# tansey/functionalmf

Measured on AMD Instinct MI355X. Metric: Gibbs sweeps/sec (full W+V update) at (512,256,64) K=5; % HBM roofline, higher is better.
Workload: dtype f64; 1 GPU; gaussian_btf c3 (512,256,64,4) nembeds=5 tf_order=2 complete data, W+V update, rng=device; burn_in_sweeps=10, step_loop=C side (btf_wv_steps: one call queues the K steps), v_sampler=spectral, likelihood_form=complete, parallelism=rows(W)/cols(V) x1

## Files before the change

### functionalmf_amd/_native.py

```python
import ctypes as C
import os
import subprocess
import sys

import numpy as np

HERE = os.path.dirname(os.path.abspath(__file__))
ROOT = os.path.dirname(HERE)
CSRC = os.path.join(HERE, "csrc")
LIB_PATH = os.environ.get("BTF_LIB_PATH") or os.path.join(HERE, "libbtf_hip.so")
UNITS = [(os.path.join(CSRC, "btf_%s.hip" % name), suffix) for name, suffix in [
    ("abi", "_abi.o"), ("analysis", "_analysis.o"), ("criteria", "_crit.o"), ("nmf", "_nmf.o"), ("gass_ep", "_gass_ep.o"),
    ("gamma_grid", "_gamma_grid.o"), ("diag", "_diag.o"), ("predict", "_predict.o"), ("functionals", "_functionals.o"),
    ("fold_in", "_fold_in.o"), ("loo", "_loo.o"), ("ranking", "_ranking.o"), ("assoc", "_assoc.o"), ("monotone", "_monotone.o"),
    ("gg_criteria", "_gg_criteria.o"), ("gg_predict", "_gg_predict.o")]]
SOURCES = [src for src, _ in UNITS]
HEADERS = sorted(os.path.join(CSRC, f) for f in os.listdir(CSRC) if f.endswith(".h")) + \
    [os.path.join(ROOT, "include", "btf.h")]

BTF_OK, BTF_EINVAL, BTF_EHIP, BTF_ENOTPD, BTF_ESTATE = 0, 1, 2, 3, 4
COMPAT = {"reference": 0, "exact": 1}
KERNEL_NAMES = ["stats", "w_accum", "w_solve", "v_accum", "v_banded", "gram", "products", "sse", "pg_draw", "nb_loglik",
                "prior_band", "gram_eig", "hyper", "ess", "criteria"]
COMM_ID_BYTES = 128
# ... 72 lines not shown
                                          _c_ip, C.c_int] + [_c_dp] * 10 + [C.c_longlong]),
    "btf_posterior_monotone": (C.c_int, [C.c_int] * 6 + [_c_dp, _c_dp, C.c_int, C.c_int, _c_dp, C.c_int, _c_dp, _c_ip, _c_dp, _c_dp]),
    "btf_collect_monotone": (C.c_int, [_ctx, C.c_int, _c_dp, _c_dp, C.c_int, C.c_int, C.c_int, _c_dp, C.c_int, _c_dp, _c_ip, _c_dp, _c_dp]),
    "btf_fold_in_rows": (C.c_int, [C.c_int] * 7 + [_c_dp] * 7 + [C.c_uint64, C.c_int, C.c_int64, _c_dp, _c_dp, C.c_int, _c_dp, C.c_int,
                                   _c_dp, _c_dp]),
    "btf_collect_fold_in": (C.c_int, [_ctx, C.c_int, C.c_int, C.c_int] + [_c_dp] * 4 + [C.c_uint64, C.c_int, C.c_int64, _c_dp, _c_dp,
                                                                                       C.c_int, _c_dp, C.c_int, _c_dp, _c_dp]),
    "btf_diag_eval": (C.c_int, [C.c_int, C.c_int, C.c_int, C.c_int, C.c_int, C.c_int, C.c_int, C.POINTER(_c_dp), C.POINTER(_c_dp),
                                C.POINTER(_ctx), C.c_int, _c_dp]),
    "btf_collect_begin": (C.c_int, [_ctx, C.c_int]),
    "btf_collect": (C.c_int, [_ctx, C.c_int]),
    "btf_collect_schedule": (C.c_int, [_ctx, C.c_int, C.c_int, C.c_int]),
    "btf_collect_end": (C.c_int, [_ctx, C.c_int, _c_dp, _c_dp, _c_dp, _c_dp]),
    "btf_collect_summary": (C.c_int, [_ctx, C.c_int, C.c_int, _c_dp, C.c_int, _c_dp, _c_dp]),
    "btf_crit_set_data": (C.c_int, [_ctx, C.c_int, _c_dp, _c_dp, _c_dp, _c_dp]),
    "btf_crit_set_logsum": (C.c_int, [_ctx, C.c_int, _c_dp]),
    "btf_crit_eval": (C.c_int, [_ctx, C.c_int, C.c_int, C.c_double, C.c_int, _c_dp, _c_dp, _c_dp, C.c_int, _c_dp, _c_dp, _c_dp]),
    "btf_crit_loo": (C.c_int, [_ctx, C.c_int, C.c_int, C.c_double, C.c_int, _c_dp, _c_dp, _c_dp, C.c_int, _c_dp, C.c_int, _c_dp, _c_dp,
                               _c_dp]),
    "btf_predict_batch": (C.c_int, [C.c_int, C.c_int, C.c_int64, _c_dp, _c_dp, C.c_uint64, _c_dp]),
    "btf_predict_eval": (C.c_int, [_ctx, C.c_int, C.c_double, C.c_int, _c_dp, _c_dp, _c_dp, C.c_int, _c_dp, _c_dp, C.c_int, C.c_int,
                                   C.c_uint64, _c_dp, C.c_int, _c_ip, C.c_int] + [_c_dp] * 11),
    "btf_predict_gg_eval": (C.c_int, [_ctx, C.c_int, _c_dp, _c_dp, _c_dp, C.c_int, C.c_int, C.c_uint64, _c_dp, C.c_int, _c_ip, C.c_int] +
                            [_c_dp] * 11),
    "btf_predict_gg_batch": (C.c_int, [C.c_int, C.c_int64, _c_dp, C.c_int, _c_dp, _c_dp, _c_dp, C.c_uint64, _c_dp, _c_ip]),
    "btf_nmf_create": (C.c_int, [C.POINTER(C.c_void_p), C.c_int, C.c_int, C.c_int, C.c_int, C.c_int, C.c_int, _c_dp,
                                 C.POINTER(C.c_uint8), C.c_double]),
    "btf_nmf_run": (C.c_int, [C.c_void_p, _c_dp, _c_dp, C.c_int, C.c_int, C.c_int, C.c_int, C.c_double, C.c_int, _c_ip, _c_dp,
                              _c_dp]),
    "btf_nmf_set_bounds": (C.c_int, [C.c_void_p, C.c_double]),
    "btf_nmf_set_row_features": (C.c_int, [C.c_void_p, C.c_int, _c_dp, C.POINTER(C.c_uint8)]),
    "btf_nmf_run_bounded": (C.c_int, [C.c_void_p, _c_dp, _c_dp, _c_dp, C.c_int, C.c_int, C.c_int, C.c_int, C.c_double, C.c_int,
                                      _c_ip, _c_dp, _c_dp, C.POINTER(C.c_uint8), _c_ip]),
    "btf_nmf_destroy": (None, [C.c_void_p]),
    "btf_nmf_pav": (C.c_int, [C.c_int, C.c_int, C.c_int, C.c_int, C.c_int, _c_dp, _c_dp]),
    "btf_sync": (C.c_int, [_ctx]),
    "btf_ess_begin": (C.c_int, [_ctx, C.c_int, _c_dp, C.c_uint64, C.c_double, C.c_int]),
    "btf_ess_eval": (C.c_int, [_ctx, C.c_int, C.c_double, C.c_int, C.c_int, _c_dp]),
    "btf_ess_run": (C.c_int, [_ctx, C.c_int, C.c_int, C.c_int, _c_dp, C.c_uint64, C.c_int, C.c_double, C.c_int]),
    "btf_ess_info": (C.c_int, [_ctx, _c_ip, _c_dp]),
    "btf_mvn_banded": (C.c_int, [C.c_int, C.c_int, C.c_int, C.c_int, _c_dp, _c_dp, _c_dp, C.c_uint64,
                                 C.c_double, C.c_int, _c_dp, _c_ip]),
    "btf_set_profiling": (C.c_int, [_ctx, C.c_int]),
    "btf_kernel_times": (C.c_int, [_ctx, _c_dp, C.POINTER(C.c_int64)]),
    "btf_set_tuning": (C.c_int, [_ctx, C.c_int, C.c_int]),
    "btf_set_option": (C.c_int, [_ctx, C.c_int, C.c_int]),
    "btf_sym_eig": (C.c_int, [C.c_int, C.c_int, C.c_int, _c_dp, _c_dp, _c_dp]),
    "btf_read_probe": (C.c_int, [C.c_int, C.c_size_t, C.c_int, _c_dp]),
    "btf_queue_Tau2": (C.c_int, [_ctx, C.c_uint64, C.c_double]),
    "btf_queue_lam2": (C.c_int, [_ctx, C.c_uint64, C.c_int]),
    "btf_gibbs_sweeps": (C.c_int, [_ctx, C.c_int, C.c_uint64, C.c_uint64, C.c_int, C.c_double, C.c_double, C.c_double,
                                   C.c_double, C.c_double, C.c_double, C.c_int]),
    "btf_wv_steps": (C.c_int, [_ctx, C.c_int, C.c_uint64, C.c_uint64, C.c_int, C.c_double, C.c_int]),
    "btf_gass_set_constraints": (C.c_int, [_ctx, _c_dp, C.c_int, _c_dp, C.c_int]),
    "btf_gass_begin": (C.c_int, [_ctx, C.c_int, C.c_int, _c_dp, _c_dp, C.c_uint64, C.c_double, C.c_int, C.c_int]),
    "btf_gass_grid": (C.c_int, [_ctx, C.c_int, _c_ip, C.POINTER(C.c_uint8), _c_dp, _c_dp]),
    "btf_gass_eval": (C.c_int, [_ctx, C.c_int, _c_dp, _c_ip, _c_dp]),
    "btf_gass_commit": (C.c_int, [_ctx, C.c_int, _c_dp, _c_ip]),
    "btf_gass_select": (C.c_int, [_ctx, C.c_int, C.c_uint64, _c_ip]),
    "btf_gass_run": (C.c_int, [_ctx, C.c_int, C.c_int, C.c_uint64, C.c_int, C.c_double, C.c_int]),
    "btf_gass_set_ep": (C.c_int, [_ctx, _c_dp, _c_dp]),
    "btf_gass_set_row_features": (C.c_int, [_ctx, C.c_int, C.POINTER(C.c_uint8), _c_dp]),
    "btf_gass_set_U": (C.c_int, [_ctx, _c_dp]),
    "btf_gass_get_U": (C.c_int, [_ctx, _c_dp]),
    "btf_mvn_dense": (C.c_int, [C.c_int, C.c_int, C.c_int, _c_dp, C.c_int, _c_dp, _c_dp, _c_dp, C.c_uint64, C.c_double, C.c_int,
                                _c_dp, _c_ip]),
    "btf_get_likelihood_form": (C.c_int, [_ctx, _c_ip]),
    "btf_get_draw_counters": (C.c_int, [_ctx, C.POINTER(C.c_uint64), C.POINTER(C.c_uint64)]),
    "btf_set_draw_counters": (C.c_int, [_ctx, C.c_uint64, C.c_uint64]),
    "btf_get_accum_bytes_per_cell": (C.c_int, [_ctx, _c_dp]),
    "btf_get_V_sampler": (C.c_int, [_ctx, _c_ip]),
    "btf_queue_scalars": (C.c_int, [_ctx, C.c_uint64, C.c_int, C.c_double, C.c_double, C.c_double, C.c_double, _c_ip]),
    "btf_host_selftest": (C.c_int, []),
    "btf_set_likelihood_param": (C.c_int, [_ctx, C.c_int, C.c_double]),
    "btf_set_likelihood_table": (C.c_int, [_ctx, C.c_int, _c_dp, _c_dp, _c_dp, C.c_int]),
    "btf_set_data_logsum": (C.c_int, [_ctx, _c_dp, _c_dp, C.c_int]),
    "btf_comm_fork": (C.c_int, [_ctx, C.c_void_p]),
    "btf_comm_join": (C.c_int, [_ctx, C.c_void_p]),
    "btf_comm_unique_id": (C.c_int, [C.POINTER(C.c_ubyte), C.c_int]),
    "btf_comm_block": (C.c_int, [C.c_int, C.c_int, C.c_int, _c_ip, _c_ip]),
    "btf_comm_init": (C.c_int, [_ctx, C.c_int, C.c_int, C.POINTER(C.c_ubyte), C.c_int]),
    "btf_comm_rehearse": (C.c_int, [_ctx, C.c_int, C.c_int]),
    "btf_peer_export": (C.c_int, [_ctx, C.POINTER(C.c_ubyte), C.c_int]),
    "btf_peer_init": (C.c_int, [_ctx, C.c_int, C.c_int, C.POINTER(C.c_ubyte), C.c_int]),
    "btf_comm_destroy": (C.c_int, [_ctx]),
    "btf_comm_info": (C.c_int, [_ctx, _c_ip]),
    "btf_allgather_W": (C.c_int, [_ctx]),
    "btf_allgather_V": (C.c_int, [_ctx]),
    "btf_allreduce_sse": (C.c_int, [_ctx]),
    "btf_allreduce_sum": (C.c_int, [_ctx, _c_dp, C.c_int]),
    "btf_set_gathered_W": (C.c_int, [_ctx, _c_dp]),
    "btf_set_gathered_V": (C.c_int, [_ctx, _c_dp]),
}


class BTFError(RuntimeError):
    def __init__(self, code, msg, index=-1):
        super().__init__("btf error %d: %s" % (code, msg))
        self.code = code
        self.index = index


class NotPositiveDefiniteError(BTFError, np.linalg.LinAlgError):
    """Raised where the reference raises LinAlgError (W step, factor.py:357) and
    where it would loop forever after the jitter retries (fast_mvn.py:69-72)."""

# ... 114 lines not shown
```

### functionalmf_amd/csrc/btf_abi.hip

```cpp
#include "../../include/btf.h"
#include "btf_kernels.h"
#include "btf_banded_fast.h"
#include "btf_banded_twist.h"
#include "btf_banded_chunk.h"
#include "btf_spectral.h"
#include "btf_gass.h"
#include "btf_gass_ep.h"
#include "btf_gass_features.h"
#include "btf_gamma_grid.h"
#include "btf_fused.h"
#include "btf_functionals.h"
#include "btf_instances.h"
#include "btf_comm.h"
#include "btf_ctx.h"
#include <hip/hip_ext.h>
#include <unistd.h>

#include <algorithm>
#include <atomic>
#include <climits>
#include <cmath>
#include <cstdio>
#include <cstdlib>
#include <cstring>
// ... 134 lines not shown
      if (cnt > VS_MAXE) { c->st_dense_ok = false; break; }
      for (int u = 0; u < cnt; ++u) { drow[e * VS_MAXE + u] = row[ptr[e] + u]; dcoef[e * VS_MAXE + u] = coef[ptr[e] + u]; }
    }
    if ((rc = dev_alloc(c, &c->st_drow, drow.size()))) return rc;
    if ((rc = dev_alloc(c, &c->st_dcoef, dcoef.size()))) return rc;
    HIPCHK(c, hipMemcpy(c->st_drow, drow.data(), drow.size() * sizeof(int), hipMemcpyHostToDevice));
    HIPCHK(c, hipMemcpy(c->st_dcoef, dcoef.data(), dcoef.size() * sizeof(double), hipMemcpyHostToDevice));
  }
  return BTF_OK;
}

inline int unr3_min_rpb() {
  static const int v = [] { const char* e = std::getenv("BTF_UNR3_RPB"); return e ? std::atoi(e) : 2048; }();
  return v;
}
inline bool lean_on() {
  static const bool v = [] { const char* e = std::getenv("BTF_ACC_LEAN"); return !e || std::atoi(e) != 0; }();
  return v;
}
template <int K>
void launch_accum(btf_ctx* c, int kid, int mode, const double* X, const double* Cx, const unsigned char* C8, const double* U,
                  const int* srcmap, int Rdim, int ld, int rpb, int nch, EigSide side = EigSide{nullptr, 0, 0, nullptr},
                  EigSideCols sidec = EigSideCols{nullptr, 0, CurveLists{nullptr, nullptr, nullptr}, nullptr, 0.0, nullptr},
                  TauSide tau = TauSide{}, GramSide gram = GramSide{},
                  ChunkMap cm = ChunkMap{0, 0, INT_MAX, 0, 0, 0}, SweepSide sw = SweepSide{},
                  const FuseW* fw = nullptr, const FuseV* fv = nullptr) {
  if (cm.row_end == 0) cm.row_end = Rdim;
  {
    static const double min_mb = [] { const char* e = std::getenv("BTF_NT_MIN_MB"); return e ? std::atof(e) : 100.0; }();
    cm.nt = (double)Rdim * (double)ld * 8.0 >= min_mb * 1048576.0 ? 1 : 0;
  }
#ifdef BTF_ACC_STAMPS
  cm.stamps = c->acc_stamps;
#endif
  Prof p(c, kid);
  const int cpw = TAU_SIDE_CPW;
  cm.nside = (sw.sc.hyp ? 1 : 0) + (sw.lam.hyp ? 1 : 0) + (side.out ? 1 + eig_side_groups(sidec.ncols, acc_waves(K, mode)) : 0) +
             (tau.Tau2 ? (tau.M + cpw - 1) / cpw : 0) + (gram.gpart ? gram.nblocks : 0) + (gram.sum_src ? 1 : 0) + (fw ? fw->owners : 0);
  dim3 grid((ld / ACC_TILE) * nch + cm.nside);
  if (fw || fv) {
    const bool unr3 = rpb >= unr3_min_rpb();
    if constexpr (K == 8) {
      if (unr3 && fw) { p.launch(accum_kernel<K, 0, 16, double, double, 3, 2, FUSE_W>, grid, dim3(16 * WAVE), 0, X, Cx, U, srcmap, c->part, Rdim, ld, rpb, side, sidec, tau, gram, cm, sw, *fw); return; }
      if (unr3 && fv) { p.launch(accum_kernel<K, 0, 16, double, double, 3, 2, FUSE_V>, grid, dim3(16 * WAVE), 0, X, Cx, U, srcmap, c->part, Rdim, ld, rpb, side, sidec, tau, gram, cm, sw, *fv); return; }
    }
    if constexpr (K <= 8) {
      if (fw) p.launch(accum_kernel<K, 0, 16, double, double, 0, 2, FUSE_W>, grid, dim3(16 * WAVE), 0, X, Cx, U, srcmap, c->part, Rdim, ld, rpb, side, sidec, tau, gram, cm, sw, *fw);
      else {
        const bool df_on = c->fused_dataflow != 0;
        FuseV f2 = *fv;
        constexpr int RG = K < 4 ? 4 : (K > 6 ? 6 : K);
        f2.dataflow = (df_on && f2.a.pband && f2.pimg && !f2.cnt && !f2.hp.flag && K <= 6 &&
                       vf_df_fits(f2.a.T, K, f2.a.TF, f2.a.nD, 16, RG)) ? 1 : 0;

        if constexpr (K <= 6) {
          if (f2.dataflow) { p.launch(accum_kernel<K, 0, 16, double, double, 0, 2, FUSE_VDF>, grid, dim3(16 * WAVE), 0, X, Cx, U, srcmap, c->part, Rdim, ld, rpb, side, sidec, tau, gram, cm, sw, f2); return; }
        }
        p.launch(accum_kernel<K, 0, 16, double, double, 0, 2, FUSE_V>, grid, dim3(16 * WAVE), 0, X, Cx, U, srcmap, c->part, Rdim, ld, rpb, side, sidec, tau, gram, cm, sw, f2);
      }
    }
    return;
  }
  const signed char* A8 = (mode >= 1 && !C8 && X == c->A_wT) ? c->A8_wT : ((mode >= 1 && !C8 && X == c->A_v) ? c->A8_v : nullptr);
  if (A8) {
    if (mode == 2) p.launch(accum_kernel<K, 2, acc_waves(K, 2), double, signed char>, grid, dim3(acc_waves(K, 2) * WAVE), 0, A8, Cx, U, srcmap, c->part, Rdim, ld, rpb, side, sidec, tau, gram, cm, sw, FuseNone{});
    else p.launch(accum_kernel<K, 1, acc_waves(K, 1), double, signed char>, grid, dim3(acc_waves(K, 1) * WAVE), 0, A8, Cx, U, srcmap, c->part, Rdim, ld, rpb, side, sidec, tau, gram, cm, sw, FuseNone{});
    return;
  }
  if (mode >= 1 && C8) {
    if (mode == 2) p.launch(accum_kernel<K, 2, acc_waves(K, 2), unsigned char>, grid, dim3(acc_waves(K, 2) * WAVE), 0, X, C8, U, srcmap, c->part, Rdim, ld, rpb, side, sidec, tau, gram, cm, sw, FuseNone{});
    else p.launch(accum_kernel<K, 1, acc_waves(K, 1), unsigned char>, grid, dim3(acc_waves(K, 1) * WAVE), 0, X, C8, U, srcmap, c->part, Rdim, ld, rpb, side, sidec, tau, gram, cm, sw, FuseNone{});
  } else if (mode == 2) p.launch(accum_kernel<K, 2>, grid, dim3(acc_waves(K, 2) * WAVE), 0, X, Cx, U, srcmap, c->part, Rdim, ld, rpb, side, sidec, tau, gram, cm, sw, FuseNone{});
  else if (mode == 1) p.launch(accum_kernel<K, 1>, grid, dim3(acc_waves(K, 1) * WAVE), 0, X, Cx, U, srcmap, c->part, Rdim, ld, rpb, side, sidec, tau, gram, cm, sw, FuseNone{});
  else if (K <= 8 && acc_waves(K, 0) == 16 && rpb < unr3_min_rpb() && !tau.Tau2 && !sw.sc.hyp && !sw.lam.hyp && lean_on()) {
    if constexpr (K <= 8) p.launch(accum_kernel<K, 0, 16, double, double, 0, 2, FUSE_LEAN>, grid, dim3(16 * WAVE), 0, X, Cx, U, srcmap, c->part, Rdim, ld, rpb, side, sidec, tau, gram, cm, sw, FuseNone{});
  }
  else if (K >= 10 && ACC_WAVES != acc_waves(10, 0) && !side.out && rpb < unr3_min_rpb()) {
    if constexpr (K >= 10) p.launch(accum_kernel<K, 0, ACC_WAVES>, grid, dim3(ACC_WAVES * WAVE), 0, X, Cx, U, srcmap, c->part, Rdim, ld, rpb, side, sidec, tau, gram, cm, sw, FuseNone{});
  }
  else if (rpb >= unr3_min_rpb()) p.launch(accum_kernel<K, 0, acc_waves(K, 0), double, double, 3>, grid, dim3(acc_waves(K, 0) * WAVE), 0, X, Cx, U, srcmap, c->part, Rdim, ld, rpb, side, sidec, tau, gram, cm, sw, FuseNone{});
  else p.launch(accum_kernel<K, 0>, grid, dim3(acc_waves(K, 0) * WAVE), 0, X, Cx, U, srcmap, c->part, Rdim, ld, rpb, side, sidec, tau, gram, cm, sw, FuseNone{});
}
struct PgPasses { bool flat, series, frac; int mode; };
PgPasses pg_passes(const btf_ctx* c) {
  PgPasses p{false, false, false, c->pg_mode};
  if (c->counts && p.mode == PG_MODE_DEFAULT) p.mode = PG_MODE_SERIES_ALL;
  if (p.mode == PG_MODE_SERIES_ALL) { p.series = true; return p; }
  if (p.mode == PG_MODE_EXACT_ALL) { p.flat = c->pg_has_small || c->pg_has_big; p.frac = c->pg_has_frac; }
  else { p.flat = c->pg_has_small; p.series = c->pg_has_big || c->pg_has_frac; }
  if (!p.flat && !p.series && !p.frac) p.series = true;
  return p;
}
template <int K>
void launch_pg(btf_ctx* c, const double* B, double* out, const double* Lf, const double* Uf, int nl, int ld, int Rdim,
               unsigned long long base, unsigned long long stride_r, unsigned long long stride_l, unsigned long long seed) {
  const int gx = (nl + PG_THREADS - 1) / PG_THREADS;
  int nrb = std::max(1, std::min(Rdim, 4096 / std::max(1, gx)));
  const int rpb = (Rdim + nrb - 1) / nrb;
  nrb = (Rdim + rpb - 1) / rpb;
  const PgPasses ps = pg_passes(c);
  int fill = 1;
  if (ps.flat) {
    Prof p(c, BTF_K_PG);
    const int rpx = round_up(rpb, PGX_CPL);
    p.launch(pgx_kernel<K, PGX_CPL>, dim3(gx, (Rdim + rpx - 1) / rpx), dim3(256), pgx_rows_lds(PGX_CPL), B, out, Lf, Uf, nl, ld, Rdim,
             rpx, base, stride_r, stride_l, seed, ps.mode, fill);
    fill = 0;
  }
  if (ps.series) {
    Prof p(c, BTF_K_PG);
    p.launch(pg_kernel<K, PG_PATH_SERIES>, dim3(gx, nrb), dim3(PG_THREADS), 0, B, out, Lf, Uf, nl, ld, Rdim, rpb, base, stride_r, stride_l, seed, ps.mode, fill);
    fill = 0;
  }
  if (ps.frac) {
    Prof p(c, BTF_K_PG);
    p.launch(pg_kernel<K, PG_PATH_EXACT>, dim3(gx, nrb), dim3(PG_THREADS), 0, B, out, Lf, Uf, nl, ld, Rdim, rpb, base, stride_r, stride_l, seed, ps.mode, fill);
  }
}
template <int K>
void launch_gram(btf_ctx* c, const double* U, int Rdim) {
  Prof p(c, BTF_K_GRAM);
  c->ngp_gram = gram_blocks(Rdim);
  p.launch(gram_kernel<K>, dim3(c->ngp_gram), dim3(GRAM_THREADS), 0, U, Rdim, c->gpart);
}
template <int K>
void launch_wsolve(btf_ctx* c, const WSolveArgs& a0) {
  Prof p(c, BTF_K_W_SOLVE);
  WSolveArgs a = a0;
  const int rw = ws_rows_for(a.nl);
  a.nside = (a.lam.hyp ? 1 : 0) + (a.band.pband ? a.band.ml : 0);
  const dim3 grid((a.nl + rw - 1) / rw + a.nside);
#define WS_LAUNCH(WT, RWV) p.launch(w_solve_kernel<K, WT, RWV>, grid, dim3(WS_ROWS * ws_split_of(K, WT)), 0, a)
#define WS_PICK(WT) do { if (rw == 8) WS_LAUNCH(WT, 8); else if (rw == 16) WS_LAUNCH(WT, 16); else if (rw == 32) WS_LAUNCH(WT, 32); else WS_LAUNCH(WT, 64); } while (0)
  if (a.weighted) WS_PICK(true); else WS_PICK(false);
#undef WS_PICK
#undef WS_LAUNCH
}
template <int K>
hipError_t launch_vbanded(btf_ctx* c, const VBandArgs& a, size_t lds_bytes) {
  static std::atomic<unsigned long long> attr_set{0};
  if (!dev_flag_is_set(attr_set, c->dev)) {
    hipError_t e = hipFuncSetAttribute((const void*)v_banded_kernel<K>, hipFuncAttributeMaxDynamicSharedMemorySize, 160 * 1024);
    if (e != hipSuccess) return e;
    dev_flag_set(attr_set, c->dev);
  }
  Prof p(c, BTF_K_V_BANDED);
  p.launch(v_banded_kernel<K>, dim3(a.ml), dim3(WAVE), lds_bytes, a);
  return hipSuccess;
}
template <int NPL, bool ROW16>
hipError_t launch_vbanded_fast(btf_ctx* c, const VBandArgs& a, size_t lds_bytes) {
  static std::atomic<unsigned long long> attr_set{0};
  if (!dev_flag_is_set(attr_set, c->dev)) {
    hipError_t e = hipFuncSetAttribute((const void*)v_banded_fast_kernel<NPL, ROW16>,
                                       hipFuncAttributeMaxDynamicSharedMemorySize, 160 * 1024);
    if (e != hipSuccess) return e;
    dev_flag_set(attr_set, c->dev);
  }
  Prof p(c, BTF_K_V_BANDED);
  p.launch(v_banded_fast_kernel<NPL, ROW16>, dim3(a.ml), dim3(VB_THREADS), lds_bytes, a, c->K);
  return hipSuccess;
}
hipError_t dispatch_vbanded_fast(btf_ctx* c, const VBandArgs& a, int bw, size_t lds_bytes, bool* handled) {
  const int npairs = bw * (bw - 1) / 2;
  const int npl = std::max(1, (npairs + WAVE - 1) / WAVE);
  *handled = true;
  if (bw <= 15) {
    if (npl == 1) return launch_vbanded_fast<1, true>(c, a, lds_bytes);
    if (npl == 2) return launch_vbanded_fast<2, true>(c, a, lds_bytes);
  } else {
    switch (npl) {
      case 2: return launch_vbanded_fast<2, false>(c, a, lds_bytes);
      case 3: return launch_vbanded_fast<3, false>(c, a, lds_bytes);
      case 4: return launch_vbanded_fast<4, false>(c, a, lds_bytes);
      case 5: return launch_vbanded_fast<5, false>(c, a, lds_bytes);
      case 6: return launch_vbanded_fast<6, false>(c, a, lds_bytes);
      case 7: return launch_vbanded_fast<7, false>(c, a, lds_bytes);
      case 8: return launch_vbanded_fast<8, false>(c, a, lds_bytes);
      default: break;
    }
  }
  *handled = false;
  return hipSuccess;
// ... 320 lines not shown
  }
  HIPCHK(c, hipStreamSynchronize(c->stream));
  if (want_sums) {
    std::vector<double> h((size_t)blocks * 3);
    HIPCHK(c, hipMemcpy(h.data(), c->bsum, h.size() * sizeof(double), hipMemcpyDeviceToHost));
    double ssw = 0.0, nobs = 0.0, sa2 = 0.0;
    for (int b = 0; b < blocks; ++b) { ssw += h[3 * b]; nobs += h[3 * b + 1]; sa2 += h[3 * b + 2]; }
    c->ssw = ssw;
    c->nobs = nobs;
    c->sa2 = sa2;
  }
  if (keep && !last) { keep->h = hY; keep->h2 = hY2; keep->d = dY; keep->d2 = dY2; }
  else {
    (void)hipFree(dY);
    if (dY2) (void)hipFree(dY2);
    if (keep) *keep = Uploaded{};
  }
  return BTF_OK;
}

int upload_relayout(btf_ctx* c, const double* h, int rows, int cols, double* dst, int ld, bool transposed) {
  const size_t cells = (size_t)rows * cols;
  double* d = nullptr;
  int rc;
  if ((rc = dev_alloc(c, &d, cells))) return rc;
  HIPCHK(c, hipMemcpy(d, h, cells * sizeof(double), hipMemcpyHostToDevice));
  const int blocks = (int)std::min<size_t>(4096, (cells + 255) / 256);
  hipLaunchKernelGGL(relayout_kernel, dim3(blocks), dim3(256), 0, c->stream, d, rows, cols, dst, ld, transposed ? 1 : 0, 1);
  HIPCHK(c, hipStreamSynchronize(c->stream));
  (void)hipFree(d);
  return BTF_OK;
}

}

extern "C" {

int btf_create(btf_ctx** out, int nrows, int ncols, int ndepth, int nembeds, int tf_order, int device, void* stream) {
  if (!out) return BTF_EINVAL;
  *out = nullptr;
  if (nrows < 1 || ncols < 1 || ndepth < 2 || nembeds < 1 || nembeds > MAX_K || tf_order < 0 || tf_order > 3)
    return fail(nullptr, BTF_EINVAL, "unsupported dims (need 1<=nembeds<=10, 0<=tf_order<=3, ndepth>=2)");
  if ((tf_order + 1) * nembeds > 63) return fail(nullptr, BTF_EINVAL, "half-bandwidth (tf_order+1)*nembeds must be <= 63");
  btf_ctx* c = new btf_ctx();
  c->N = nrows; c->M = ncols; c->T = ndepth; c->K = nembeds; c->TF = tf_order; c->KK = tri(nembeds);
  c->dev = device;
  c->row0 = 0; c->nl = nrows; c->col0 = 0; c->ml = ncols;
  if (int rc = use_device(device)) { delete c; return rc; }
  { int n = 0; if (hipDeviceGetAttribute(&n, hipDeviceAttributeMultiprocessorCount, device) == hipSuccess && n > 0) c->ncu = n; }
  { const char* e = std::getenv("BTF_FUSED_STEP"); if (e) c->fused_step = std::max(0, std::min(2, std::atoi(e))); }
  { const char* e = std::getenv("BTF_LAM_IN_WSOLVE"); if (e) c->lam_in_wsolve = std::atoi(e) != 0; }
  { const char* e = std::getenv("BTF_BAND_IN_WSOLVE"); if (e) c->band_in_wsolve = std::atoi(e) != 0; }
  { const char* e = std::getenv("BTF_VF_DATAFLOW"); if (e) c->fused_dataflow = std::atoi(e) != 0 ? 1 : 0; }
  if (stream) { c->stream = (hipStream_t)stream; }
  else {
    const hipError_t e = hipStreamCreateWithFlags(&c->stream, hipStreamNonBlocking);
    if (e != hipSuccess) { g_err = std::string("hipStreamCreate: ") + hipGetErrorString(e); delete c; return BTF_EHIP; }
    c->own_stream = true;
  }
  int rc = BTF_OK;
  auto A = [&](int r) { if (rc == BTF_OK) rc = r; };
  A(dev_alloc(c, &c->W, (size_t)(nrows + 64) * nembeds));
  A(dev_alloc(c, &c->V, (size_t)(ncols + 64) * ndepth * nembeds));
  A(dev_alloc(c, &c->gpart, (size_t)GRAM_BLOCKS * c->KK));
  A(dev_alloc(c, &c->status, 4));
  if (rc == BTF_OK) {
    int init[4] = {0, -1, 0, 0};
    if (hipMemcpy(c->status, init, sizeof(init), hipMemcpyHostToDevice) != hipSuccess) rc = BTF_EHIP;
  }
  if (rc == BTF_OK) rc = build_stencil(c);
  A(dev_alloc(c, &c->Tau2, (size_t)ncols * c->nD));
  A(dev_alloc(c, &c->tries, (size_t)ncols));
  if (rc != BTF_OK) { std::string m = c->err; btf_destroy(c); g_err = m; return rc; }
  *out = c;
  return BTF_OK;
}

void btf_destroy(btf_ctx* c) {
  if (!c) return;
  (void)hipSetDevice(c->dev);
  if (c->stream) (void)hipStreamSynchronize(c->stream);
  void* ptrs[] = {c->A_wT, c->C_wT, c->A_v, c->C_v, c->B_wT, c->B_v, c->W, c->V, c->Tau2, c->part,
                  c->gpart, c->zbuf, c->bsum, c->gband, c->status, c->tries, c->st_ptr, c->st_row, c->st_coef,
                  c->srcmap_w, c->srcmap_v, c->pband, c->pimg, c->dbg, c->gpart_w, c->gpart_v, c->gsum_v, c->eig, c->cv_cptr, c->cv_crow, c->cv_cdef, c->cv_rptr, c->cv_rcol, c->cv_rdef, c->eig_cols, c->cv_dcols, c->A8_wT, c->A8_v, c->gs_cons, c->gs_cc, c->gs_rc, c->gs_av, c->gs_mask, c->gs_info, c->gs_thetas, c->gs_ntheta, c->gs_ll, c->gs_llp, c->gs_hh, c->gs_cur, c->gs_nacc, c->gs_u, c->st_drow, c->st_dcoef, c->essX0, c->essNu, c->ess_st, c->ess_theta, c->ess_done, c->ess_part, c->Ta, c->Tb, c->Tc, c->lsum, c->dr_ptr, c->dr_col, c->dr_val, c->sse_cols, c->vs_rec, c->vc_scratch, c->gs_cptr, c->gs_cidx, c->gs_cval,
                  c->ep_rows, c->ep_cols, c->ep_crow, c->ep_ccol, c->ep_mu, c->ep_corr, c->ep_pband, c->ep_envg, c->ep_f, c->ep_off,
                  c->gg_tab, c->gg_Lw, c->gg_Lv,
                  c->ft_rows, c->ft_cols, c->ft_U, c->ft_side, c->ft_X0, c->ft_Nu, c->ft_z, c->ft_mask, c->ft_info, c->ft_thetas,
                  c->ft_ntheta, c->ft_ll, c->ft_hh, c->ft_cur, c->ft_part, c->ft_nacc, c->ft_u, c->ft_theta, c->ft_keep};
  for (void* p : ptrs) if (p) (void)hipFree(p);
  if (c->pin) (void)hipHostFree(c->pin);
  if (c->pin_lsum) (void)hipHostFree(c->pin_lsum);
  if (c->pin_hyp) (void)hipHostFree(c->pin_hyp);
  for (void* p : {(void*)c->nb_data, (void*)c->nb_S, (void*)c->nb_cnt, (void*)c->nb_R, (void*)c->nb_C, (void*)c->nb_tmp, (void*)c->nb_out, (void*)c->nb_H, (void*)c->nb_Hd, (void*)c->nb_Hs, (void*)c->nb_G, (void*)c->nb_L, (void*)c->nb_optr, (void*)c->nb_oval, (void*)c->fill_tab, (void*)c->C8_wT, (void*)c->C8_v, (void*)c->smp_W, (void*)c->smp_V, (void*)c->smp_T, (void*)c->smp_s})
    if (p) (void)hipFree(p);
  for (int sl = 0; sl < 2; ++sl)
    for (void* p : {(void*)c->crit_S1[sl], (void*)c->crit_cnt[sl], (void*)c->crit_c0[sl], (void*)c->crit_c1[sl], (void*)c->crit_L[sl]})
      if (p) (void)hipFree(p);
  if (c->hyp) (void)hipFree(c->hyp);
  if (c->fz_words) (void)hipFree(c->fz_words);
  if (c->fz_pub) (void)hipFree(c->fz_pub);
  for (auto& e : c->ev_pool) { (void)hipEventDestroy(e.a); (void)hipEventDestroy(e.b); }
  if (c->ev_draw) (void)hipEventDestroy(c->ev_draw);
  if (c->ev_join) (void)hipEventDestroy(c->ev_join);
  (void)btf_comm_destroy(c);

  if (c->own_stream && c->stream) (void)hipStreamDestroy(c->stream);
  delete c;
}

const char* btf_last_error(const btf_ctx* c) { return c ? c->err.c_str() : g_err.c_str(); }
int btf_fail_index(const btf_ctx* c) { return c ? c->fail_index : fold_fail_index(); }

int btf_set_shard(btf_ctx* c, int row0, int nrows_local, int col0, int ncols_local) {
  if (!c) return BTF_EINVAL;
  if (c->have_data) return fail(c, BTF_ESTATE, "btf_set_shard must precede btf_set_data_*");
  if (row0 < 0 || nrows_local < 0 || row0 + nrows_local > c->N || col0 < 0 || ncols_local < 0 || col0 + ncols_local > c->M)
    return fail(c, BTF_EINVAL, "shard out of range");
  c->row0 = row0; c->nl = nrows_local; c->col0 = col0; c->ml = ncols_local;
  c->hrow = c->hcol = -1;
  ++c->prior_version;
  if (c->pband) { (void)hipFree(c->pband); c->pband = nullptr; c->pband_version = 0; }
  if (c->pimg) { (void)hipFree(c->pimg); c->pimg = nullptr; c->pimg_version = 0; }
  c->v_wants_band = false;
  c->nb_bwt_written = false;
  return BTF_OK;
}
int btf_set_shard_halo(btf_ctx* c, int halo_row, int halo_col) {
  if (!c) return BTF_EINVAL;
  if (halo_row < -1 || halo_row >= c->N || halo_col < -1 || halo_col >= c->M) return fail(c, BTF_EINVAL, "halo source out of range");
  if ((halo_row >= c->row0 && halo_row < c->row0 + c->nl) || (halo_col >= c->col0 && halo_col < c->col0 + c->ml))
    return fail(c, BTF_EINVAL, "halo source inside the shard's own block");
  if (halo_row != c->hrow || halo_col != c->hcol) {
    c->have_data = false;
    c->nb_bwt_written = false;
  }
  c->hrow = halo_row; c->hcol = halo_col;
  return BTF_OK;
}
void* btf_stream(btf_ctx* c) { return c ? (void*)c->stream : nullptr; }
void* btf_dev_W(btf_ctx* c) { return c ? c->W : nullptr; }
void* btf_dev_V(btf_ctx* c) { return c ? c->V : nullptr; }

static int detect_curve_counts(btf_ctx* c) {
  c->curve = false;
  c->cv_cij.clear();
  if (!c->C8_v || c->nl != c->N || c->ml != c->M) return BTF_OK;
  const int N = c->N, M = c->M, T = c->T;
  std::vector<unsigned char> h((size_t)N * c->ldv);
  HIPCHK(c, hipMemcpy(h.data(), c->C8_v, h.size(), hipMemcpyDeviceToHost));
  std::vector<unsigned char> cij((size_t)N * M);
  for (int i = 0; i < N; ++i)
    for (int j = 0; j < M; ++j) {
      const unsigned char* p = h.data() + (size_t)i * c->ldv + (size_t)j * T;
      const unsigned char v = p[0];
      for (int t = 1; t < T; ++t) if (p[t] != v) return BTF_OK;
      cij[(size_t)i * M + j] = v;
    }
  std::vector<int> cptr(M + 1, 0), rptr(N + 1, 0);
  size_t nnz = 0;
  for (int i = 0; i < N; ++i)
    for (int j = 0; j < M; ++j) if (cij[(size_t)i * M + j] < c->R) { ++cptr[j + 1]; ++rptr[i + 1]; ++nnz; }
  if (nnz == 0 || nnz > (size_t)N * M / 4) return BTF_OK;
  for (int j = 0; j < M; ++j) cptr[j + 1] += cptr[j];
  for (int i = 0; i < N; ++i) rptr[i + 1] += rptr[i];
  std::vector<int> crow(nnz), rcol(nnz), cfill(cptr.begin(), cptr.end() - 1), rfill(rptr.begin(), rptr.end() - 1);
  std::vector<double> cdef(nnz), rdef(nnz);
  for (int i = 0; i < N; ++i)
    for (int j = 0; j < M; ++j) {
      const int v = cij[(size_t)i * M + j];
      if (v >= c->R) continue;
      const double d = (double)(c->R - v);
      crow[cfill[j]] = i; cdef[cfill[j]++] = d;
      rcol[rfill[i]] = j; rdef[rfill[i]++] = d;
    }
  int rc;
  if ((rc = dev_alloc(c, &c->cv_cptr, cptr.size()))) return rc;
// ... 151 lines not shown
      if (src_col[c->col0 + jl] == c->hcol) s = c->ml;
      else if (s < 0 || s >= c->ml) return fail(c, BTF_EINVAL, "stale weight source column outside this shard: declare it with btf_set_shard_halo before the upload (or use compat=exact)");
      if (s != jl && c->curve) {
        bool same = true;
        for (int i = 0; i < c->N && same; ++i) same = c->cv_cij[(size_t)i * c->M + jl] == c->cv_cij[(size_t)i * c->M + s];
        if (same) continue;
      }
      for (int t = 0; t < c->T; ++t) mv[jl * c->T + t] = s * c->T + t;
      c->stale_v |= (s != jl);
    }
  if ((rc = dev_alloc(c, &c->srcmap_w, mw.size()))) return rc;
  if ((rc = dev_alloc(c, &c->srcmap_v, mv.size()))) return rc;
  HIPCHK(c, hipMemcpy(c->srcmap_w, mw.data(), mw.size() * sizeof(int), hipMemcpyHostToDevice));
  HIPCHK(c, hipMemcpy(c->srcmap_v, mv.data(), mv.size() * sizeof(int), hipMemcpyHostToDevice));
  return BTF_OK;
}

int btf_set_W(btf_ctx* c, const double* W) {
  if (!c || !W) return BTF_EINVAL;
  HIPCHK(c, hipSetDevice(c->dev));
  HIPCHK(c, hipMemcpyAsync(c->W, W, (size_t)c->N * c->K * sizeof(double), hipMemcpyHostToDevice, c->stream));
  HIPCHK(c, hipStreamSynchronize(c->stream));
  c->have_W = true;
  c->nb_L_valid = false;
  c->ngp_w = 0;
  c->v_local_done = false;
  c->sse_cols_valid = false;
  return BTF_OK;
}
int btf_set_gathered_W(btf_ctx* c, const double* W) {
  if (!c) return BTF_EINVAL;
  const bool keep = c->v_local_done;
  const int rc = btf_set_W(c, W);
  if (rc == BTF_OK) c->v_local_done = keep;
  return rc;
}
int btf_get_W(btf_ctx* c, double* W) {
  if (!c || !W) return BTF_EINVAL;
  HIPCHK(c, hipSetDevice(c->dev));
  HIPCHK(c, hipMemcpyAsync(W, c->W, (size_t)c->N * c->K * sizeof(double), hipMemcpyDeviceToHost, c->stream));
  return check_status(c);
}
int btf_set_V(btf_ctx* c, const double* V) {
  if (!c || !V) return BTF_EINVAL;
  HIPCHK(c, hipSetDevice(c->dev));
  HIPCHK(c, hipMemcpyAsync(c->V, V, (size_t)c->M * c->T * c->K * sizeof(double), hipMemcpyHostToDevice, c->stream));
  HIPCHK(c, hipStreamSynchronize(c->stream));
  c->have_V = true;
  c->nb_L_valid = false;
  c->w_part_valid = false;
  c->ngp_v = 0;
  c->w_local_done = false;
  c->sse_cols_valid = false;
  return BTF_OK;
}
int btf_set_gathered_V(btf_ctx* c, const double* V) {
  if (!c) return BTF_EINVAL;
  const bool keep = c->w_local_done;
  const int rc = btf_set_V(c, V);
  if (rc == BTF_OK) c->w_local_done = keep;
  return rc;
}
int btf_get_V(btf_ctx* c, double* V) {
  if (!c || !V) return BTF_EINVAL;
  HIPCHK(c, hipSetDevice(c->dev));
  HIPCHK(c, hipMemcpyAsync(V, c->V, (size_t)c->M * c->T * c->K * sizeof(double), hipMemcpyDeviceToHost, c->stream));
  return check_status(c);
}
int btf_set_hyper(btf_ctx* c, const double* Tau2, double lam2, double sigma2) {
  if (!c) return BTF_EINVAL;
  HIPCHK(c, hipSetDevice(c->dev));
  if (Tau2) {
    HIPCHK(c, hipMemcpyAsync(c->Tau2, Tau2, (size_t)c->M * c->nD * sizeof(double), hipMemcpyHostToDevice, c->stream));
    HIPCHK(c, hipStreamSynchronize(c->stream));
    c->have_hyper = true;
  }
  if (Tau2 || lam2 != c->lam2) ++c->prior_version;
  c->lam2 = lam2; c->sigma2 = sigma2;
  return BTF_OK;
}
int btf_set_tau_chain(btf_ctx* c, const double* Ta, const double* Tb, const double* Tc) {
  if (!c || !Ta || !Tb || !Tc) return BTF_EINVAL;
  HIPCHK(c, hipSetDevice(c->dev));
  const size_t n = (size_t)c->M * c->nD;
  int rc;
  if (!c->Ta) {
    if ((rc = dev_alloc(c, &c->Ta, n))) return rc;
    if ((rc = dev_alloc(c, &c->Tb, n))) return rc;
    if ((rc = dev_alloc(c, &c->Tc, n))) return rc;
    if ((rc = dev_alloc(c, &c->lsum, (size_t)c->M))) return rc;
  }
  HIPCHK(c, hipMemcpyAsync(c->Ta, Ta, n * sizeof(double), hipMemcpyHostToDevice, c->stream));
  HIPCHK(c, hipMemcpyAsync(c->Tb, Tb, n * sizeof(double), hipMemcpyHostToDevice, c->stream));
  HIPCHK(c, hipMemcpyAsync(c->Tc, Tc, n * sizeof(double), hipMemcpyHostToDevice, c->stream));
  HIPCHK(c, hipStreamSynchronize(c->stream));
  c->have_chain = true;
  return BTF_OK;
}

int btf_get_tau(btf_ctx* c, double* Tau2, double* Ta, double* Tb, double* Tc) {
  if (!c || !Tau2) return BTF_EINVAL;
  HIPCHK(c, hipSetDevice(c->dev));
  const size_t n = (size_t)c->M * c->nD * sizeof(double);
  HIPCHK(c, hipMemcpyAsync(Tau2, c->Tau2, n, hipMemcpyDeviceToHost, c->stream));
  if (Ta && c->Ta) {
    HIPCHK(c, hipMemcpyAsync(Ta, c->Ta, n, hipMemcpyDeviceToHost, c->stream));
// ... 220 lines not shown
      if (gram.gpart) {
        gram.cnt = c->fz_words + FZ_GRAM;
        c->fz_gram_total += (unsigned)gram.nblocks;
        fw.gram_cnt = gram.cnt; fw.gram_expected = c->fz_gram_total;
      }
      c->fz_w_total += (unsigned)nch_total;
      fw.expected = c->fz_w_total;
      fw.rows = own_rows;
      fw.owners = tiles * (ACC_TILE / own_rows);
    }
    K_SWITCH(K, launch_accum<KT>(c, BTF_K_W_ACCUM, mode, c->A_wT, c->C_wT, c->C8_wT, c->V, c->srcmap_w, MT, c->ldw, rpb, nch_launch,
                                 EigSide{nullptr, 0, 0, nullptr}, EigSideCols{nullptr, 0, CurveLists{nullptr, nullptr, nullptr}, nullptr, 0.0, nullptr}, tau, gram, cm, sw,
                                 fuse ? &fw : nullptr));
    if (fuse) {
      wf->done = true;
      const int wrows = ws_rows_for(c->nl);
      c->ngp_w = fw.a.gout ? (c->nl + wrows - 1) / wrows : 0;
      c->ngp_v = 0;
    }
    c->tau_pending = false;
  } else if (c->tau_pending && c->dev_scalars && c->have_chain) {
    Prof p(c, BTF_K_HYPER);
    p.launch(tau2_kernel, dim3(c->M), dim3(256), 0, tau_side_of(c, c->tau_seed, 1.0, c->tau_stability), c->K);
    c->tau_pending = false;
  }
  HIPCHK(c, hipGetLastError());
  c->w_part_valid = true; c->w_part_mode = mode; c->w_part_nch = nch_total; c->w_part_rpb = rpb; c->w_part_gv = use_gv;
  c->w_part_curve = cv;
  return BTF_OK;
}
}

namespace {
int v_accum_local(btf_ctx* c, int compat);
int mark_draw(btf_ctx* c);
}

int btf_w_accum(btf_ctx* c, int compat) {
  if (!c) return BTF_EINVAL;
  if (!c->have_data || !c->have_V || !c->have_W) return fail(c, BTF_ESTATE, "set data, W and V first");
  HIPCHK(c, hipSetDevice(c->dev));
  return w_accum_phase(c, compat);
}

int btf_resample_W(btf_ctx* c, const double* z, uint64_t seed, int compat) {
  if (!c) return BTF_EINVAL;
  if (!c->have_data || !c->have_V || !c->have_W) return fail(c, BTF_ESTATE, "set data, W and V first");
  HIPCHK(c, hipSetDevice(c->dev));
  const int K = c->K, KK = c->KK;
  const bool wt = lik_weighted(c), cv = c->weighted && !wt;
  const int want_mode = !wt ? 0 : (compat == BTF_COMPAT_REFERENCE && c->stale_w && c->srcmap_w ? 2 : 1);
  int rc;
  c->v_local_done = false;
  const double* dz = nullptr;
  if (z) {
    const size_t nz = (size_t)w_z_offset(c->N, K);
    if ((rc = ensure_z(c, nz))) return rc;
    HIPCHK(c, hipMemcpyAsync(c->zbuf, z, nz * sizeof(double), hipMemcpyHostToDevice, c->stream));
    dz = c->zbuf;
  }
  WFuseReq wf{dz, seed, false};
  if (!(c->w_part_valid && c->w_part_mode == want_mode && c->w_part_curve == cv)) { if ((rc = w_accum_phase(c, compat, ACC_ALL, &wf))) return rc; }
  if (c->sc_pending) return fail(c, BTF_ESTATE, "btf_queue_scalars must be followed by the W accumulation that carries it");
  const int nch = c->w_part_nch;
  const bool use_gv = c->w_part_gv;
  c->w_part_valid = false;
  if (c->nl > 0 && !wf.done) {
    const bool whole = c->nl == c->N && c->ml == c->M;
    WSolveArgs a{};
    a.part = c->part; a.nch = nch; a.ld = c->ldw; a.weighted = wt ? 1 : 0;
    a.gsrc = (wt && want_mode == 2) ? c->srcmap_w : nullptr;
    a.gpart = use_gv ? c->gpart_v : c->gpart; a.ngp = use_gv ? c->ngp_v : c->ngp_gram;
    if (use_gv && c->w_part_gsum) { a.gpart = c->gsum_v; a.ngp = 1; }
    const int wrows = ws_rows_for(c->nl);
    const int wblocks = (c->nl + wrows - 1) / wrows;
    if (whole && c->fuse_gram) {
      if (!c->gpart_w) { if ((rc = dev_alloc(c, &c->gpart_w, (size_t)std::max(64, (c->N + WS_ROWS - 1) / WS_ROWS) * KK))) return rc; }
      a.gout = c->gpart_w;
    }
    a.s = c->binomial ? 1.0 : 1.0 / c->nu2;
    a.sR = a.s * c->R;
    a.inv_sigma2 = 1.0 / c->sigma2;
    a.hyp = c->dev_scalars ? c->hyp : nullptr; a.Rrep = c->R; a.hyp_noise = c->binomial ? 0 : 1;
    a.W = c->W; a.row0 = c->row0; a.nl = c->nl;
#ifdef BTF_WS_STAMPS
    a.dbg = c->dbg;
#endif
    a.z = dz; a.seed = seed; a.stream = 2 * c->sweep_w + 0x10000ULL;
    a.status = c->status;
    if (cv) { a.cv = CurveLists{c->cv_rptr, c->cv_rcol, c->cv_rdef}; a.cv_blocks = c->gpart_v; }
    if (c->lam_in_wsolve && c->lam_pending && c->dev_scalars && c->lsum && c->have_chain) {
      a.lam = LamSide{c->lsum, c->M, (double)c->nD * c->M * c->K + 1.0, c->lam_exact, c->lam_seed, c->hyp, nullptr, nullptr, 0u};
      c->lam_pending = false;
      ++c->prior_version;
      const int TD1 = c->T * (c->TF + 2);
      if (c->band_in_wsolve && c->v_wants_band && c->pband && (!c->band_img || c->pimg) && TD1 <= 2 * WS_ROWS * ws_split_of(K, wt) &&
          c->nD <= 2 * WS_ROWS * ws_split_of(K, wt)) {
        if ((rc = ensure_fused(c))) return rc;
        ++c->fz_epoch;
        a.lam.pub = c->fz_pub + FZ_PUB_HYP; a.lam.flag = c->fz_words + FZ_LAM; a.lam.epoch = c->fz_epoch;
        a.band = BandSide{c->Tau2, c->nD, c->st_ptr, c->st_row, c->st_coef, TD1, c->col0, c->ml, c->pband,
                          c->band_img ? c->pimg : nullptr, c->T, c->TF + 2, c->band_PB, nullptr, 0.0,
                          c->fz_pub + FZ_PUB_HYP, c->fz_words + FZ_LAM, c->fz_epoch, c->status};
        c->pband_version = c->prior_version;
        c->pimg_version = c->band_img ? c->prior_version : 0;
      }
    }
    K_SWITCH(K, launch_wsolve<KT>(c, a));
    c->ngp_w = a.gout ? wblocks : 0;
    c->ngp_v = 0;
  }
  c->sweep_w++;
  c->nb_L_valid = false;
  c->sse_cols_valid = false;
  HIPCHK(c, hipGetLastError());
  if (split_applies(c)) {
    if ((rc = mark_draw(c))) return rc;
    return v_accum_local(c, compat);
  }
  return BTF_OK;
}

static int v_banded_dispatch(btf_ctx* c, int choice, const double* dz, uint64_t seed, int nch, bool use_gw, double eps0,
                             int attempts, double* out, bool prior_only) {
  const int K = c->K, KK = c->KK, T = c->T, n = T * K;
  const bool wt = lik_weighted(c), cv = c->weighted && !wt && !prior_only;
  const bool whole = c->nl == c->N && c->ml == c->M;
  int rc;
  const int bw = (c->TF + 1) * K, R1 = bw + 1, D1 = c->TF + 2;
  size_t lds_fixed = (size_t)(3 * n + T * D1 + (wt ? T * KK : KK) + (bw * (bw + 1) / 2 + 3) / 4) * sizeof(double);
  size_t lds_band = std::max((size_t)n * R1, (size_t)(GRAM_BLOCKS + 16) * KK) * sizeof(double);
  size_t lds_bytes = lds_fixed + lds_band;
  VBandArgs a{};
  if (lds_bytes > 150 * 1024) {
    if (wt) lds_fixed -= (size_t)T * KK * sizeof(double);
    if (lds_fixed > 150 * 1024) return fail(c, BTF_EINVAL, "ndepth*nembeds too large for the on-chip vectors");
    const size_t stride = (size_t)n * R1 + (wt ? (size_t)T * KK : 0);
    if (!c->gband || c->gband_stride != stride) {
      if ((rc = dev_alloc(c, &c->gband, (size_t)c->ml * stride))) return rc;
      c->gband_stride = stride;
    }
    a.gband = c->gband; a.gband_stride = c->gband_stride;
    lds_bytes = lds_fixed;
  }
  a.part = c->part; a.nch = nch; a.ld = c->ldv; a.weighted = wt ? 1 : 0;
  a.gsrc = (wt && c->v_part_mode == 2) ? c->srcmap_v : nullptr;
  a.gpart = use_gw ? c->gpart_w : c->gpart; a.ngp = use_gw ? c->ngp_w : c->ngp_gram;
  a.s = c->binomial ? 1.0 : 1.0 / c->nu2;
  a.sR = a.s * c->R;
  a.Tau2 = c->Tau2; a.lam2 = c->lam2; a.nD = c->nD;
  a.hyp = c->dev_scalars ? c->hyp : nullptr; a.Rrep = c->R; a.hyp_noise = c->binomial ? 0 : 1;
  a.panel4 = c->sampler == BTF_SAMPLER_BANDED_NOPANEL ? 0 : 1;
  a.st_ptr = c->st_ptr; a.st_row = c->st_row; a.st_coef = c->st_coef;
  a.T = T; a.TF = c->TF; a.col0 = c->col0; a.ml = c->ml;
  a.V = c->V; a.z = dz; a.seed = seed; a.stream = 2 * c->sweep_v + 0x10001ULL;
  a.eps0 = eps0; a.attempts = attempts; a.status = c->status; a.tries = c->tries; a.dbg = c->dbg;
  if (prior_only) { a.nch = 0; a.ngp = 0; a.s = 0.0; a.sR = 0.0; a.hyp_noise = 0; }
  if (cv) { a.cv = CurveLists{c->cv_cptr, c->cv_crow, c->cv_cdef}; a.cv_W = c->W; }
  a.V = out;
// ... 64 lines not shown
    }
  }
  if (!handled) { a.gout = nullptr; if (!prior_only) c->ngp_v = 0; }
  if (!handled) { K_SWITCH(K, e = launch_vbanded<KT>(c, a, lds_bytes)); }
  HIPCHK(c, e);
  return BTF_OK;
}

namespace {
int v_accum_local(btf_ctx* c, int compat) {
  c->v_local_done = false;
  if (!split_applies(c)) return BTF_OK;
  const int K = c->K, KK = c->KK;
  const bool wt = lik_weighted(c);
  const int mode = !wt ? 0 : (compat == BTF_COMPAT_REFERENCE && c->stale_v && c->srcmap_v ? 2 : 1);
  if (mode == 2) return BTF_OK;
  const int NV = wt ? K + KK : K;
  const int tiles = c->ldv / ACC_TILE;
  const int rpb = pick_rpb(c->N, tiles, c->rpb_v, wt, acc_slots(c, K, mode), v_side_reserve(c, wt));
  const int nch = (c->N + rpb - 1) / rpb;
  const SplitGeom sg = split_geom(c->row0, c->row0 + c->nl, c->N, rpb, tiles);
  if (!sg.ok) return BTF_OK;
  int rc;
  if ((rc = ensure_part(c, (size_t)std::max(nch, sg.nch_r + sg.nch_l) * NV * c->ldv))) return rc;
  K_SWITCH(K, launch_accum<KT>(c, BTF_K_V_ACCUM, mode, c->A_v, c->C_v, c->C8_v, c->W, c->srcmap_v, c->N, c->ldv, sg.rpb_l, sg.nch_l,
                               EigSide{nullptr, 0, 0, nullptr}, EigSideCols{nullptr, 0, CurveLists{nullptr, nullptr, nullptr}, nullptr, 0.0, nullptr},
                               TauSide{}, GramSide{}, ChunkMap{sg.nch_r, sg.lo, INT_MAX, 0, sg.hi, 0}));
  HIPCHK(c, hipGetLastError());
  c->v_local_done = true; c->v_local_rpb = rpb; c->v_local_mode = mode;
  return BTF_OK;
}
int mark_draw(btf_ctx* c) {
  if (!c->ev_draw) HIPCHK(c, hipEventCreateWithFlags(&c->ev_draw, hipEventDisableTiming));
  HIPCHK(c, hipEventRecord(c->ev_draw, c->stream));
  return BTF_OK;
}
int after_v_draw(btf_ctx* c, int compat) {
  if (!split_applies(c)) return BTF_OK;
  int rc;
  if ((rc = mark_draw(c))) return rc;
  return w_accum_phase(c, compat, ACC_LOCAL);
}
}

int btf_resample_V(btf_ctx* c, const double* z, uint64_t seed, int compat, double eps0, int attempts) {
  if (!c) return BTF_EINVAL;
  if (!c->have_data || !c->have_V || !c->have_W || !c->have_hyper) return fail(c, BTF_ESTATE, "set data, W, V and hyper-parameters first");
  if (attempts < 0) attempts = 0;
  HIPCHK(c, hipSetDevice(c->dev));
  c->w_local_done = false;
  c->sse_cols_valid = false;
  struct ResetFlag { bool& f; ~ResetFlag() { f = false; } } reset_nu2_flag{c->nu2_drawn_since_v};
  const int K = c->K, KK = c->KK, T = c->T, n = T * K;
  const bool wt = lik_weighted(c), cv = c->weighted && !wt;
  const int mode = !wt ? 0 : (compat == BTF_COMPAT_REFERENCE && c->stale_v && c->srcmap_v ? 2 : 1);
  c->v_part_mode = mode;
  const int NV = wt ? K + KK : K;
  const int tiles = c->ldv / ACC_TILE;
  const int rpb = pick_rpb(c->N, tiles, c->rpb_v, wt, acc_slots(c, K, mode), v_side_reserve(c, wt));
  const SplitGeom vsg = split_applies(c) ? split_geom(c->row0, c->row0 + c->nl, c->N, rpb, tiles) : SplitGeom{};
  const bool v_rest_only = c->v_local_done && vsg.ok && c->v_local_rpb == rpb && c->v_local_mode == mode;
  c->v_local_done = false;
  const int nch_all = (c->N + rpb - 1) / rpb;
  const int nch = v_rest_only ? vsg.nch_r + vsg.nch_l : nch_all;
  int rc;
  if ((rc = ensure_part(c, (size_t)nch * NV * c->ldv))) return rc;
  const double* dz = nullptr;
  if (z) {
    const size_t nz = (size_t)c->M * n;
    if ((rc = ensure_z(c, nz))) return rc;
    HIPCHK(c, hipMemcpyAsync(c->zbuf, z, nz * sizeof(double), hipMemcpyHostToDevice, c->stream));
    dz = c->zbuf;
  }
  if (c->ml > 0) {
    const bool whole = c->nl == c->N && c->ml == c->M;
    const bool use_gw = !wt && whole && c->fuse_gram && c->ngp_w > 0;
    const int choice = banded_choice(c);
    const bool gram_aside = !wt && !use_gw && choice == 3 && c->N <= 16384;
    if (!wt && !use_gw && !gram_aside) { K_SWITCH(K, launch_gram<KT>(c, c->W, c->N)); }
    EigSide side{nullptr, 0, 0, nullptr};
    if (choice == 3) {
      if (!c->eig) {
        if ((rc = dev_alloc(c, &c->eig, (size_t)K + K * K + 8))) return rc;
        HIPCHK(c, hipMemsetAsync(c->eig, 0, ((size_t)K + K * K + 8) * sizeof(double), c->stream));
      }
      side = EigSide{use_gw ? c->gpart_w : c->gpart, use_gw ? c->ngp_w : c->ngp_gram, K, c->eig, gram_aside ? c->W : nullptr, c->N};
    }
    EigSideCols sidec{nullptr, 0, CurveLists{nullptr, nullptr, nullptr}, nullptr, 0.0, nullptr};
    const bool cols_aside = choice == 3 && cv;
    if (cols_aside) sidec = EigSideCols{c->cv_dcols, c->cv_ndef, CurveLists{c->cv_cptr, c->cv_crow, c->cv_cdef}, c->W, 1.0 / c->R, c->eig_cols};
    const bool fuse_v = c->fused_step >= 1 && choice == 3 && !wt && !cv && mode == 0 && c->TF == 2 && K <= 8 && !v_rest_only && !split_applies(c) &&
                        vf_fits(T, K, c->TF, c->nD, 16, rpb >= unr3_min_rpb()) && vs_lds_bytes(T, K, c->TF, c->nD, false) <= 160 * 1024 &&
                        !(rpb >= unr3_min_rpb() && K != 8);
    const ChunkMap cm = v_rest_only ? ChunkMap{0, 0, vsg.lo, vsg.hi - vsg.lo, c->N, 0} : ChunkMap{0, 0, INT_MAX, 0, c->N, 0};
    SweepSide sw{};
    if (c->lam_pending && c->dev_scalars && c->lsum && c->have_chain) {
      sw.lam = LamSide{c->lsum, c->M, (double)c->nD * c->M * c->K + 1.0, c->lam_exact, c->lam_seed, c->hyp};
      c->lam_pending = false;
      ++c->prior_version;
    }
    if (!fuse_v) {
      K_SWITCH(K, launch_accum<KT>(c, BTF_K_V_ACCUM, mode, c->A_v, c->C_v, c->C8_v, c->W, c->srcmap_v, c->N, c->ldv, rpb,
                                   v_rest_only ? vsg.nch_r : nch_all, side, sidec, TauSide{}, GramSide{}, cm, sw));
    }
    hipError_t e = hipSuccess;
    if (choice == 3) {
// ... 30 lines not shown
      if (rg) {
        const size_t need = (size_t)c->ml * n * (c->TF + 3);
        if (need > c->vs_rec_elems) { if ((rc = dev_alloc(c, &c->vs_rec, need))) return rc; c->vs_rec_elems = need; }
        sa.rec_g = c->vs_rec;
        const int TD1 = T * (c->TF + 2);
        if (!c->pband) { if ((rc = dev_alloc(c, &c->pband, (size_t)c->ml * TD1))) return rc; }
        {
          Prof p(c, BTF_K_PRIOR);
          p.launch(prior_band_kernel, dim3((c->ml * TD1 + 255) / 256), dim3(256), 0, (const double*)c->Tau2, c->lam2, c->nD,
                   (const int*)c->st_ptr, (const int*)c->st_row, (const double*)c->st_coef, TD1, c->col0, c->ml, c->pband,
                   (const double*)(c->dev_scalars ? c->hyp : nullptr), 0, (double*)nullptr, 0, 0, 0);
        }
        c->pband_version = 0;
        sa.pband = c->pband;
      }
      if (fuse_v) {
        if ((rc = ensure_fused(c))) return rc;
        ++c->fz_epoch;
        FuseV fv{};
        fv.a = sa;
        if (!sw.lam.hyp) {
          const int TD1 = T * (c->TF + 2);
          if (!c->pband) { if ((rc = dev_alloc(c, &c->pband, (size_t)c->ml * TD1))) return rc; c->pband_version = 0; }
          const bool img = c->TF == 2 && K <= 6 && vf_df_fits(T, K, c->TF, c->nD, 16, K < 4 ? 4 : K);
          const int PB = df_layout(T, K, c->TF + 1).PB;
          if (img && !c->pimg) {
            if ((rc = dev_alloc(c, &c->pimg, (size_t)c->ml * 2 * PB))) return rc;
            HIPCHK(c, hipMemsetAsync(c->pimg, 0, (size_t)c->ml * 2 * PB * sizeof(double), c->stream));
            c->pimg_version = 0;
          }
          c->v_wants_band = true; c->band_img = img; c->band_PB = PB;
          if (c->pband_version != c->prior_version || (img && c->pimg_version != c->prior_version)) {
            Prof p(c, BTF_K_PRIOR);
            if (TD1 <= 512 && c->nD <= 256)
              p.launch(prior_band_cols_kernel, dim3(c->ml), dim3(256), 0, (const double*)c->Tau2, c->lam2, c->nD,
                       (const int*)c->st_ptr, (const int*)c->st_row, (const double*)c->st_coef, TD1, c->col0, c->pband,
                       (const double*)(c->dev_scalars ? c->hyp : nullptr), img ? c->pimg : (double*)nullptr, T, c->TF + 2, PB);
            else
              p.launch(prior_band_kernel, dim3((c->ml * TD1 + 255) / 256), dim3(256), 0, (const double*)c->Tau2, c->lam2, c->nD,
                       (const int*)c->st_ptr, (const int*)c->st_row, (const double*)c->st_coef, TD1, c->col0, c->ml, c->pband,
                       (const double*)(c->dev_scalars ? c->hyp : nullptr), 1, img ? c->pimg : (double*)nullptr, T, c->TF + 2, PB);
            c->pband_version = c->prior_version;
            c->pimg_version = img ? c->prior_version : 0;
          }
          fv.a.pband = c->pband;
          if (img && c->pimg_version == c->prior_version) fv.pimg = c->pimg;
        }
        fv.cnt = nch_all > 1 ? c->fz_words + FZ_TICKETS + c->fz_tiles_w : nullptr;
        { static const int be = [] { const char* e = std::getenv("BTF_BAND_EARLY"); return e ? std::atoi(e) : 0; }(); fv.band_early = be; }
        fv.eig_pub = c->fz_pub + FZ_PUB_EIG; fv.eig_flag = c->fz_words + FZ_EIG; fv.epoch = c->fz_epoch;
        side.pub = c->fz_pub + FZ_PUB_EIG; side.flag = c->fz_words + FZ_EIG; side.epoch = c->fz_epoch;
        side.gran = reinterpret_cast<unsigned long long*>(c->fz_pub + FZ_PUB_GRAN);
        fv.eig_gran = side.gran;
        if (sw.lam.hyp) {
          sw.lam.pub = c->fz_pub + FZ_PUB_HYP; sw.lam.flag = c->fz_words + FZ_LAM; sw.lam.epoch = c->fz_epoch;
          fv.hp = HypPub{c->fz_pub + FZ_PUB_HYP, c->fz_words + FZ_LAM, c->fz_epoch, 4};
        }
        K_SWITCH(K, launch_accum<KT>(c, BTF_K_V_ACCUM, mode, c->A_v, c->C_v, c->C8_v, c->W, c->srcmap_v, c->N, c->ldv, rpb,
                                     nch_all, side, sidec, TauSide{}, GramSide{}, cm, sw, nullptr, &fv));
        c->sweep_v++;
        c->nb_L_valid = false;
        c->w_part_valid = false;
        HIPCHK(c, hipGetLastError());
        return after_v_draw(c, compat);
      }
      if (!rg) {
        static const bool lazy_band = [] { const char* e2 = std::getenv("BTF_TWIST_PBAND"); return !e2 || std::atoi(e2) != 0; }();
        const int TD1 = T * (c->TF + 2);
        if (!lazy_band) { }
        else if (c->pband && c->pband_version == c->prior_version) sa.pband = c->pband;
        else if (c->last_v_prior_version == c->prior_version) {
          if (!c->pband) { if ((rc = dev_alloc(c, &c->pband, (size_t)c->ml * TD1))) return rc; }
          Prof p(c, BTF_K_PRIOR);
          p.launch(prior_band_kernel, dim3((c->ml * TD1 + 255) / 256), dim3(256), 0, (const double*)c->Tau2, c->lam2, c->nD,
                   (const int*)c->st_ptr, (const int*)c->st_row, (const double*)c->st_coef, TD1, c->col0, c->ml, c->pband,
                   (const double*)(c->dev_scalars ? c->hyp : nullptr), 1, (double*)nullptr, 0, 0, 0);
          c->pband_version = c->prior_version;
          sa.pband = c->pband;
        }
        c->last_v_prior_version = c->prior_version;
      }
      const size_t sl = vs_lds_bytes(T, K, c->TF, c->nD, rg);
      switch ((c->TF + 1) * 2 + (rg ? 1 : 0)) {
        case 2: e = launch_vspectral<1, false>(c, sa, sl); break;
        case 3: e = launch_vspectral<1, true>(c, sa, sl); break;
        case 4: e = launch_vspectral<2, false>(c, sa, sl); break;
        case 5: e = launch_vspectral<2, true>(c, sa, sl); break;
        case 6:
          switch (K) {
#define VS_FIXED(KV) case KV: e = launch_vspectral<3, false, KV>(c, sa, sl); break
            VS_FIXED(1); VS_FIXED(2); VS_FIXED(3); VS_FIXED(4); VS_FIXED(5); VS_FIXED(6); VS_FIXED(7); VS_FIXED(8); VS_FIXED(9); VS_FIXED(10);
#undef VS_FIXED
            default: e = launch_vspectral<3, false>(c, sa, sl); break;
          }
          break;
        case 7:
          switch (K) {
#define VS_FIXED(KV) case KV: e = launch_vspectral<3, true, KV>(c, sa, sl); break
            VS_FIXED(1); VS_FIXED(2); VS_FIXED(3); VS_FIXED(4); VS_FIXED(5); VS_FIXED(6); VS_FIXED(7); VS_FIXED(8); VS_FIXED(9); VS_FIXED(10);
#undef VS_FIXED
            default: e = launch_vspectral<3, true>(c, sa, sl); break;
          }
          break;
        case 8: e = launch_vspectral<4, false>(c, sa, sl); break;
        default: e = launch_vspectral<4, true>(c, sa, sl); break;
      }
// ... 711 lines not shown
  if (what == 2) return BTF_OK;
  if (what == 0) c->ngp_w = 0; else c->ngp_v = 0;
  c->w_part_valid = false; c->w_local_done = c->v_local_done = false; c->sse_cols_valid = false; c->nb_L_valid = false;
  return BTF_OK;
}

int btf_gass_select(btf_ctx* c, int what, uint64_t seed, int32_t* naccept_out) {
  if (!c) return BTF_EINVAL;
  if (c->gs_what != what || c->gs_chains < 1) return fail(c, BTF_ESTATE, "btf_gass_select follows btf_gass_begin of the same factor");
  HIPCHK(c, hipSetDevice(c->dev));
  const int nch = c->gs_chains;
  const GassBufs b = gass_bufs(c, what);
  {
    Prof p(c, BTF_K_ESS);
    p.launch(gass_select_kernel, dim3(nch), dim3(GASS_THREADS), 0, (const double*)b.ll, (const int*)b.ntheta, (const double*)b.thetas,
             (const double*)b.hh, (const double*)b.X0, (const double*)b.Nu, b.X, b.per,
             (unsigned long long)(seed * 0x9E3779B97F4A7C15ULL + 0xBB67AE8584CAA73BULL), b.nacc, (double*)nullptr,
             (const double*)(c->gs_ep ? c->ep_mu : nullptr));
  }
  HIPCHK(c, hipGetLastError());
  if (what == 0) c->ngp_w = 0; else if (what == 1) c->ngp_v = 0;
  if (what != 2) { c->w_part_valid = false; c->w_local_done = c->v_local_done = false; c->sse_cols_valid = false; c->nb_L_valid = false; }
  if (naccept_out) {
    HIPCHK(c, hipMemcpyAsync(naccept_out, b.nacc, (size_t)nch * sizeof(int), hipMemcpyDeviceToHost, c->stream));
    return check_status(c);
  }
  return BTF_OK;
}

int btf_gass_run(btf_ctx* c, int what, int link, uint64_t seed, int ngrid, double eps0, int attempts) {
  if (ngrid < 1) return fail(c, BTF_EINVAL, "ngrid must be positive");
  int rc;
  if ((rc = btf_gass_begin(c, what, link, nullptr, nullptr, seed, eps0, attempts, ngrid))) return rc;
  if ((rc = btf_gass_eval(c, what, nullptr, nullptr, nullptr))) return rc;
  return btf_gass_select(c, what, seed, nullptr);
}

int btf_gibbs_sweeps(btf_ctx* c, int n, uint64_t seed_base, uint64_t draws0, int compat, double nu2_a, double nu2_b,
                     double sigma2_a, double sigma2_b, double stability, double eps0, int attempts) {
  if (!c || n < 0) return BTF_EINVAL;
  if (!c->dev_scalars || c->binomial || c->counts) return fail(c, BTF_ESTATE, "btf_gibbs_sweeps: Gaussian data with device-resident scalars");
  if (c->nl != c->N || c->ml != c->M) return fail(c, BTF_ESTATE, "btf_gibbs_sweeps: unsharded contexts (a sharded sweep has exchanges between its steps)");
  if (!c->have_data || !c->have_W || !c->have_V || !c->have_hyper || !c->have_chain)
    return fail(c, BTF_ESTATE, "set data, W, V, the hyper-parameters and the horseshoe+ chain first");
  int rc;
  for (int s = 0; s < n; ++s) {
    const uint64_t d = seed_base + draws0 + 5ULL * (uint64_t)s;
    if ((rc = btf_queue_Tau2(c, d + 1, stability))) return rc;
    if ((rc = btf_queue_lam2(c, d + 2, compat))) return rc;
    int32_t queued = 0;
    if ((rc = btf_queue_scalars(c, d + 3, 3, nu2_a, nu2_b, sigma2_a, sigma2_b, &queued))) return rc;
    if ((rc = btf_w_accum(c, compat))) return rc;
    if (!queued) { if ((rc = btf_draw_scalars(c, d + 3, 7, nu2_a, nu2_b, sigma2_a, sigma2_b))) return rc; }
    if ((rc = btf_resample_W(c, nullptr, d + 4, compat))) return rc;
    if ((rc = btf_resample_V(c, nullptr, d + 5, compat, eps0, attempts))) return rc;
    if (c->col_every > 0 && --c->col_count == 0) {
      if ((rc = btf_collect(c, c->col_slot++))) return rc;
      c->col_count = c->col_every;
      if (c->col_slot >= c->smp_n) c->col_every = 0;
    }
  }
  return BTF_OK;
}

int btf_wv_steps(btf_ctx* c, int n, uint64_t seed_base, uint64_t draws0, int compat, double eps0, int attempts) {
  if (!c || n < 0) return BTF_EINVAL;
  if (c->nl != c->N || c->ml != c->M) return fail(c, BTF_ESTATE, "btf_wv_steps: unsharded contexts (a sharded step has an exchange behind each half-sweep)");
  if (!c->have_data || !c->have_W || !c->have_V || !c->have_hyper) return fail(c, BTF_ESTATE, "set data, W, V and hyper-parameters first");
  int rc;
  for (int s = 0; s < n; ++s) {
    const uint64_t d = seed_base + draws0 + 2ULL * (uint64_t)s;
    if ((rc = btf_resample_W(c, nullptr, d + 1, compat))) return rc;
    if ((rc = btf_resample_V(c, nullptr, d + 2, compat, eps0, attempts))) return rc;
  }
  return BTF_OK;
}

int btf_set_likelihood_param(btf_ctx* c, int family, double par) {
  if (!c || family < 0 || family >= ESS_FAM_COUNT || !(par == par)) return fail(c, BTF_EINVAL, "bad likelihood family / parameter");
  if (family == ESS_FAM_GAMMA_GRID) return fail(c, BTF_EINVAL, "the gamma-grid family takes a table: btf_set_likelihood_table");
  if ((family == ESS_FAM_GAUSSIAN || family == ESS_FAM_NEGBIN_LOGIT) && !(par > 0.0)) return fail(c, BTF_EINVAL, "the parameter must be positive");
  c->lik_par[family] = par;
  return BTF_OK;
}

int btf_set_likelihood_table(btf_ctx* c, int family, const double* shape, const double* scale, const double* prob, int G) {
  if (!c) return BTF_EINVAL;
  if (family != ESS_FAM_GAMMA_GRID) return fail(c, BTF_EINVAL, "btf_set_likelihood_table: family 5 (gamma grid) only");
  if (!shape || !scale || !prob || G < 1 || G > GG_MAXG) return fail(c, BTF_EINVAL, "the gamma grid has 1..128 components");
  std::vector<GgComp> h;
  double psum = 0.0;
  for (int g = 0; g < G; ++g) {
    const double a = shape[g], s = scale[g], p = prob[g];
    if (!std::isfinite(a) || !std::isfinite(s) || !std::isfinite(p) || !(a > 0.0) || !(s > 0.0) || !(p >= 0.0))
      return fail(c, BTF_EINVAL, "gamma grid: finite shape > 0, scale > 0 and weight >= 0 expected");
    psum += p;
    if (p > 0.0) h.push_back(GgComp{std::log(p), a, 1.0 / s, a * std::log(s) + std::lgamma(a)});
  }
  if (h.empty()) return fail(c, BTF_EINVAL, "gamma grid: every weight is zero");
  HIPCHK(c, hipSetDevice(c->dev));
  int rc;
  if ((rc = dev_alloc(c, &c->gg_tab, (size_t)GG_MAXG))) return rc;
  HIPCHK(c, hipMemcpy(c->gg_tab, h.data(), h.size() * sizeof(GgComp), hipMemcpyHostToDevice));
  c->gg_G = (int)h.size();
  c->gg_lsp = std::log(psum);
  gg_pred_table(shape, scale, prob, G, c->gg_pred, c->gg_mbar);
  return BTF_OK;
}

int btf_set_data_logsum(btf_ctx* c, const double* y_rows, const double* y_cols, int nreps) {
  if (!c || !y_rows || !y_cols || nreps < 1) return fail(c, BTF_EINVAL, "bad data arguments");
  if (!c->have_data || c->binomial || c->counts || nreps != c->R)
    return fail(c, BTF_ESTATE, "btf_set_data_logsum follows btf_set_data_gaussian with the same Y");
  HIPCHK(c, hipSetDevice(c->dev));
  const int MT = c->M * c->T;
  const int rows_w = slab_rows(c), cols_v = slab_cols(c) * c->T;
  int rc;
  if ((rc = dev_alloc(c, &c->gg_Lw, (size_t)MT * c->ldw))) return rc;
  if ((rc = dev_alloc(c, &c->gg_Lv, (size_t)c->N * c->ldv))) return rc;
  HIPCHK(c, hipMemsetAsync(c->gg_Lw, 0, (size_t)MT * c->ldw * sizeof(double), c->stream));
  HIPCHK(c, hipMemsetAsync(c->gg_Lv, 0, (size_t)c->N * c->ldv * sizeof(double), c->stream));
  int zero = 0;
  HIPCHK(c, hipMemcpy(c->status + 3, &zero, sizeof(int), hipMemcpyHostToDevice));
  double* dY = nullptr;
  auto one = [&](const double* hY, int rows, int cols, int ld, int transposed, double* L) -> int {
    const size_t n = (size_t)rows * cols * nreps;
    int r;
// ... 847 lines not shown
    ms_total[k] = c->ms_total[k];
    launches[k] = c->profiling ? timed[k] : c->launches[k];
    c->ms_total[k] = 0.0;
    c->launches[k] = 0;
  }
  c->ev_used = 0;
  return BTF_OK;
}

extern "C" int btf_debug_eig(btf_ctx* c, double* out) {
  if (!c || !out) return BTF_EINVAL;
  if (!c->eig) return fail(c, BTF_ESTATE, "no eigen-system yet");
  HIPCHK(c, hipSetDevice(c->dev));
  HIPCHK(c, hipStreamSynchronize(c->stream));
  HIPCHK(c, hipMemcpy(out, c->eig, ((size_t)c->K + c->K * c->K + 8) * sizeof(double), hipMemcpyDeviceToHost));
  return BTF_OK;
}
#ifdef BTF_ACC_STAMPS
extern "C" int btf_debug_acc_stamps(btf_ctx* c, long long* out) {
  if (!c) return BTF_EINVAL;
  HIPCHK(c, hipSetDevice(c->dev));
  HIPCHK(c, hipStreamSynchronize(c->stream));
  if (!c->acc_stamps) {
    int rc = dev_alloc(c, &c->acc_stamps, (size_t)8192 * 8);
    if (rc) return rc;
  }
  HIPCHK(c, hipMemcpy(out, c->acc_stamps, sizeof(long long) * 8192 * 8, hipMemcpyDeviceToHost));
  HIPCHK(c, hipMemset(c->acc_stamps, 0, sizeof(long long) * 8192 * 8));
  return BTF_OK;
}
#endif
extern "C" int btf_debug_stamps(btf_ctx* c, long long* out) {
  if (!c) return BTF_EINVAL;
  HIPCHK(c, hipSetDevice(c->dev));
  if (!c->dbg) {
    int rc = dev_alloc(c, &c->dbg, (size_t)c->M * 6);
    if (rc) return rc;
    HIPCHK(c, hipMemset(c->dbg, 0, (size_t)c->M * 6 * sizeof(long long)));
    return BTF_OK;
  }
  HIPCHK(c, hipStreamSynchronize(c->stream));
  HIPCHK(c, hipMemcpy(out, c->dbg, (size_t)c->ml * 6 * sizeof(long long), hipMemcpyDeviceToHost));
  return BTF_OK;
}

int btf_set_tuning(btf_ctx* c, int rows_per_block_w, int rows_per_block_v) {
  if (!c || rows_per_block_w < 0 || rows_per_block_v < 0) return fail(c, BTF_EINVAL, "rows per workgroup must be >= 0 (0 = default)");
  c->rpb_w = rows_per_block_w; c->rpb_v = rows_per_block_v;
  return BTF_OK;
}

int btf_set_option(btf_ctx* c, int option, int value) {
  if (!c) return BTF_EINVAL;
  switch (option) {
    case BTF_OPT_SAMPLER:
      if (value < BTF_SAMPLER_BANDED || value > BTF_SAMPLER_BANDED_NOPANEL) return fail(c, BTF_EINVAL, "unknown sampler");
      c->sampler = value;
      c->ngp_v = 0;
      return BTF_OK;
    case BTF_OPT_NB_HISTOGRAMS:
      c->nb_hist = value != 0;
      return BTF_OK;
    case BTF_OPT_PG_EXACT:
      if (value < PG_MODE_DEFAULT || value > PG_MODE_SERIES_ALL) return fail(c, BTF_EINVAL, "unknown Polya-Gamma mode");
      c->pg_mode = value;
      return BTF_OK;
    case BTF_OPT_FUSE_GRAM:
      c->fuse_gram = value != 0;
      c->ngp_v = c->ngp_w = 0;
      return BTF_OK;
    case BTF_OPT_FUSED_STEP:
      if (value < 0 || value > 2) return fail(c, BTF_EINVAL, "BTF_OPT_FUSED_STEP: 0, 1 or 2");
      c->fused_step = value;
      return BTF_OK;
    case BTF_OPT_FUSED_DATAFLOW:
      c->fused_dataflow = value != 0 ? 1 : 0;
      return BTF_OK;
    case BTF_OPT_FUSED_SWEEP:
      c->fused_sweep = value != 0;
      c->sse_cols_valid = false;
      return BTF_OK;
    case BTF_OPT_SPLIT_ACCUM:
      c->split_accum = value != 0;
      c->w_local_done = c->v_local_done = false; c->sse_cols_valid = false;
      return BTF_OK;
    case BTF_OPT_CURVE_COUNTS:
      c->curve_opt = value != 0;
      c->ngp_v = c->ngp_w = 0;
      c->w_part_valid = false; c->w_local_done = c->v_local_done = false; c->sse_cols_valid = false;
      return BTF_OK;
    default:
      return fail(c, BTF_EINVAL, "unknown option");
  }
}

int btf_get_likelihood_form(btf_ctx* c, int32_t* form) {
  if (!c || !form) return BTF_EINVAL;
  if (!c->have_data) return fail(c, BTF_ESTATE, "set data first");
  *form = !c->weighted ? BTF_LIK_COMPLETE : (curve_on(c) ? BTF_LIK_CURVE_COUNTS : BTF_LIK_WEIGHTED);
  return BTF_OK;
}

int btf_get_draw_counters(btf_ctx* c, uint64_t* w, uint64_t* v) {
  if (!c || !w || !v) return BTF_EINVAL;
  *w = c->sweep_w; *v = c->sweep_v;
  return BTF_OK;
}

int btf_set_draw_counters(btf_ctx* c, uint64_t w, uint64_t v) {
  if (!c) return BTF_EINVAL;
  c->sweep_w = w; c->sweep_v = v;
  c->sse_cols_valid = false;
  HIPCHK(c, hipSetDevice(c->dev));
  const size_t rec = (size_t)c->K + (size_t)c->K * c->K + 8;
  if (c->eig) HIPCHK(c, hipMemsetAsync(c->eig, 0, rec * sizeof(double), c->stream));
  if (c->eig_cols) HIPCHK(c, hipMemsetAsync(c->eig_cols, 0, (size_t)c->M * rec * sizeof(double), c->stream));
  return BTF_OK;
}

int btf_comm_fork(btf_ctx* c, void* comm_stream) {
  if (!c || !comm_stream) return BTF_EINVAL;
  HIPCHK(c, hipSetDevice(c->dev));
  int rc;
  if (!(c->ev_draw && split_applies(c))) { if ((rc = mark_draw(c))) return rc; }
  HIPCHK(c, hipStreamWaitEvent((hipStream_t)comm_stream, c->ev_draw, 0));
  return BTF_OK;
}
int btf_comm_join(btf_ctx* c, void* comm_stream) {
  if (!c || !comm_stream) return BTF_EINVAL;
  HIPCHK(c, hipSetDevice(c->dev));
  if (!c->ev_join) HIPCHK(c, hipEventCreateWithFlags(&c->ev_join, hipEventDisableTiming));
  HIPCHK(c, hipEventRecord(c->ev_join, (hipStream_t)comm_stream));
  HIPCHK(c, hipStreamWaitEvent(c->stream, c->ev_join, 0));
  return BTF_OK;
}

namespace {
#define RCCLCHK(ctx, api, call)                                                                     \
  do {                                                                                              \
    ncclResult_t r__ = (call);                                                                      \
    if (r__ != ncclSuccess)                                                                         \
      return fail(ctx, BTF_EHIP, std::string(#call) + ": " + (api)->GetErrorString(r__));           \
  } while (0)

int comm_ready(btf_ctx* c, RcclApi** api) {
  if (!c) return BTF_EINVAL;
  *api = nullptr;
  if (c->peer_on) { HIPCHK(c, hipSetDevice(c->dev)); return BTF_OK; }
  if (!c->comm) return fail(c, BTF_ESTATE, "no communicator: btf_comm_init (or btf_peer_init) first");
  std::string why;
  if (!(*api = rccl_api(&why))) return fail(c, BTF_EHIP, why);
  HIPCHK(c, hipSetDevice(c->dev));
  return BTF_OK;
}
int comm_blocks_match(btf_ctx* c) {
  const int r = c->gather_rank, w = c->gather_world;
  if (c->row0 != comm_block_lo(c->N, r, w) || c->nl != comm_block_len(c->N, r, w) ||
      c->col0 != comm_block_lo(c->M, r, w) || c->ml != comm_block_len(c->M, r, w))
    return fail(c, BTF_ESTATE, "btf_set_shard blocks are not rank " + std::to_string(r) + " of " + std::to_string(w) +
                                   "'s equal chunks ceil(n / world) (btf_comm_block)");
  return BTF_OK;
}
int peer_collective(btf_ctx* c, int which, size_t off, size_t len, const double* red_src, double* red_dst, int red_n, hipStream_t s) {
  if (c->gather_world <= 1) {
// ... 323 lines not shown
      }
    }
  const int Rs[] = {64, 512, 576, 1536, 4096, 16384, 65536}, tilesv[] = {1, 4, 64};
  for (int Rdim : Rs)
    for (int tiles : tilesv)
      for (int wt = 0; wt <= 1; ++wt)
        for (int world = 2; world <= 8; world *= 2)
          for (int rank = 0; rank < world; ++rank) {
            const int rpb = pick_rpb(Rdim, tiles, 0, wt != 0);
            ST_CHECK(rpb >= 64 && rpb % 64 == 0);
            const int chunk = (Rdim + world - 1) / world, lo = std::min(rank * chunk, Rdim), hi = std::min(lo + chunk, Rdim);
            const SplitGeom g = split_geom(lo, hi, Rdim, rpb, tiles);
            if (!g.ok) continue;
            std::vector<int> cover(Rdim, 0);
            auto walk = [&](ChunkMap cm, int rp, int nch) {
              for (int l = 0; l < nch; ++l) {
                int r0 = cm.row_base + l * rp;
                if (r0 >= cm.skip_at) r0 += cm.skip_rows;
                const int r1 = std::min(r0 + rp, cm.row_end);
                for (int r = r0; r < r1; ++r) { if (r < 0 || r >= Rdim) return false; cover[r]++; }
              }
              return true;
            };
            ST_CHECK(walk(ChunkMap{g.nch_r, g.lo, INT_MAX, 0, g.hi, 0}, g.rpb_l, g.nch_l));
            ST_CHECK(walk(ChunkMap{0, 0, g.lo, g.hi - g.lo, Rdim, 0}, rpb, g.nch_r));
            for (int v : cover) ST_CHECK(v == 1);
          }
  {
    const int rw = pick_rpb(65536, 4, 0, false, 256, 32), rv = pick_rpb(4096, 64, 0, false, 256, 1);
    ST_CHECK(rw % 64 == 0 && rv % 64 == 0);
    ST_CHECK(4 * ((65536 + rw - 1) / rw) + 32 <= 256 && 4 * ((65536 + rw - 1) / rw) + 32 > 192);
    ST_CHECK(64 * ((4096 + rv - 1) / rv) + 1 <= 256);
    ST_CHECK(pick_rpb(16384, 4, 0, false, 256, 0) == 512 && pick_rpb(512, 128, 0, false, 256, 1) == 512);
    ST_CHECK(pick_rpb(65536, 4, 0, false, 0, 0) == 1024);
  }
  {
    const int Ss[] = {1, 2, 3, 4, 63, 64, 65, 1000, 8191, 8192, 8193, 16384};
    const struct { size_t budget; int cap; } uses[] = {{SUMMARY_SORT_LDS, SUMMARY_SORT_CELLS}, {PRED_SORT_LDS, PRED_SORT_CELLS},
                                                      {(size_t)FUNC_SORT_LDS, FUNC_SORT_CELLS}};
    for (int S : Ss)
      for (const auto& u : uses) {
        const SortGeom g = sort_geom(S, u.budget, u.cap);
        const int lo = std::max(S, 2);
        ST_CHECK((g.P & (g.P - 1)) == 0 && g.P >= lo && g.P < 2 * lo);
        ST_CHECK(g.cells >= 1 && g.cells <= u.cap);
        ST_CHECK(g.lds == 8 * (size_t)g.cells * g.P && g.lds <= std::max(u.budget, 8 * (size_t)g.P));
        if (u.budget == SUMMARY_SORT_LDS) ST_CHECK(g.lds <= 128 * 1024);
      }
  }
  ST_CHECK(pg_class_of(0.0, PG_MODE_DEFAULT) == PG_CLASS_NONE && pg_class_of(4.0, PG_MODE_DEFAULT) == PG_CLASS_FLAT);
  ST_CHECK(pg_class_of(33.0, PG_MODE_DEFAULT) == PG_CLASS_SERIES && pg_class_of(33.0, PG_MODE_EXACT_ALL) == PG_CLASS_FLAT);
  ST_CHECK(pg_class_of(2.5, PG_MODE_EXACT_ALL) == PG_CLASS_FRAC && pg_class_of(2.0, PG_MODE_SERIES_ALL) == PG_CLASS_SERIES);
  ST_CHECK(pg_class_of(200.0, PG_MODE_EXACT_ALL) == PG_CLASS_NORMAL);
#undef ST_CHECK
  return 0;
}

int btf_get_accum_bytes_per_cell(btf_ctx* c, double* bytes) {
  if (!c || !bytes) return BTF_EINVAL;
  if (!c->have_data) return fail(c, BTF_ESTATE, "set data first");
  if (!lik_weighted(c)) *bytes = 8.0;
  else if (c->C8_wT) *bytes = 9.0;
  else if (c->A8_wT) *bytes = 9.0;
  else *bytes = 16.0;
  return BTF_OK;
}

int btf_get_V_sampler(btf_ctx* c, int32_t* which) {
  if (!c || !which) return BTF_EINVAL;
  const int ch = banded_choice(c);
  *which = ch == 3 ? BTF_SAMPLER_SPECTRAL : (ch == 2 ? (c->sampler == BTF_SAMPLER_BANDED_NOPANEL ? BTF_SAMPLER_BANDED_NOPANEL : BTF_SAMPLER_BANDED)
                                                     : (ch == 1 || ch == 4 ? BTF_SAMPLER_CHAIN : BTF_SAMPLER_GENERIC));
  return BTF_OK;
}

}
```

### functionalmf_amd/csrc/btf_ctx.h

```cpp
#pragma once
#include "../../include/btf.h"
#include "btf_device.h"
#include "btf_pg_exact.h"
#include "btf_gamma_grid.h"
#include "btf_scratch.h"
#include <hip/hip_ext.h>

#include <algorithm>
#include <string>
#include <vector>

typedef struct ncclComm* ncclComm_t;
namespace btf {
struct PeerMailbox; struct PeerTable;
constexpr int MAX_K = 10;
struct EvPair { hipEvent_t a, b; int kid; };
}

struct btf_ctx {
  int N = 0, M = 0, T = 0, K = 0, TF = 0, nD = 0, KK = 0;
  int dev = 0;
  int ncu = 256;
  hipStream_t stream = nullptr;
  bool own_stream = false;
  int row0 = 0, nl = 0, col0 = 0, ml = 0;
  int hrow = -1, hcol = -1;
  int ldw = 0, ldv = 0;
  int R = 1;
  bool have_data = false, binomial = false, weighted = false;
  double* A_wT = nullptr; double* C_wT = nullptr; double* A_v = nullptr; double* C_v = nullptr;
  double* B_wT = nullptr; double* B_v = nullptr;
  unsigned char* C8_wT = nullptr; unsigned char* C8_v = nullptr;
  signed char* A8_wT = nullptr; signed char* A8_v = nullptr;
  double* W = nullptr; double* V = nullptr;
  double* Tau2 = nullptr;
  double lam2 = 1.0, sigma2 = 1.0, nu2 = 1.0;
  bool have_W = false, have_V = false, have_hyper = false;
  double* part = nullptr; size_t part_elems = 0;
  double* gpart = nullptr; int ngp_gram = 16;
  double* zbuf = nullptr; size_t z_elems = 0;
  double* bsum = nullptr; size_t bsum_elems = 0;
  double* gband = nullptr; size_t gband_stride = 0;
  int* status = nullptr;
  int* tries = nullptr;
  int* st_ptr = nullptr; int* st_row = nullptr; double* st_coef = nullptr;
  int* st_drow = nullptr; double* st_dcoef = nullptr; bool st_dense_ok = false;
  int* srcmap_w = nullptr; int* srcmap_v = nullptr;
  bool stale_w = false, stale_v = false;
  int v_part_mode = 0;
  double ssw = 0.0, nobs = 0.0, sa2 = 0.0;
  double nobs_global = -1.0;
  bool w_part_valid = false; int w_part_mode = 0, w_part_nch = 0, w_part_rpb = 0; bool w_part_gv = false;
  int rpb_w = 0, rpb_v = 0;
  int sampler = BTF_SAMPLER_BANDED;
  double* eig = nullptr;
  double* essX0 = nullptr; double* essNu = nullptr; double* ess_st = nullptr; double* ess_theta = nullptr; int* ess_done = nullptr;
  double* ess_part = nullptr; size_t ess_part_elems = 0; int ess_last_chains = 0;
  double* gs_cons = nullptr; double* gs_cc = nullptr; double* gs_rc = nullptr; int gs_J = 0, gs_nrc = 0;
  int* gs_cptr = nullptr; int* gs_cidx = nullptr; double* gs_cval = nullptr; int gs_cnnz = 0;
  double* gs_av = nullptr; unsigned char* gs_mask = nullptr; int* gs_info = nullptr;
  double* gs_thetas = nullptr; int* gs_ntheta = nullptr; double* gs_ll = nullptr; double* gs_llp = nullptr; size_t gs_llp_elems = 0; double* gs_hh = nullptr; double* gs_cur = nullptr;
  int* gs_nacc = nullptr; double* gs_u = nullptr;
  int gs_chains = 0, gs_what = -1, gs_link = 0;
  int ft_F = 0; unsigned char* ft_rows = nullptr; unsigned char* ft_cols = nullptr; double* ft_U = nullptr;
  std::vector<double> gs_rc_host; double* ft_side = nullptr;
  double* ft_X0 = nullptr; double* ft_Nu = nullptr; double* ft_z = nullptr; unsigned char* ft_mask = nullptr; int* ft_info = nullptr;
  double* ft_thetas = nullptr; int* ft_ntheta = nullptr; double* ft_ll = nullptr; double* ft_hh = nullptr; double* ft_cur = nullptr;
  double* ft_part = nullptr; int* ft_nacc = nullptr; double* ft_u = nullptr; double* ft_theta = nullptr; int* ft_keep = nullptr;
  double2* ep_rows = nullptr; double2* ep_cols = nullptr; double* ep_crow = nullptr; double* ep_ccol = nullptr;
// ... 29 lines not shown
  int nb_ymax = 0;
  double* nb_G = nullptr;
  bool nb_tabulable = false;
  bool nb_L_valid = false;
  bool nb_hist = true;
  int pg_mode = btf::PG_MODE_DEFAULT;
  bool pg_has_small = true, pg_has_big = true, pg_has_frac = true;
  double* smp_W = nullptr; double* smp_V = nullptr; double* smp_T = nullptr; double* smp_s = nullptr; int smp_n = 0;
  double* crit_S1[2] = {nullptr, nullptr}; double* crit_cnt[2] = {nullptr, nullptr};
  double* crit_c0[2] = {nullptr, nullptr}; double* crit_c1[2] = {nullptr, nullptr};
  double* crit_L[2] = {nullptr, nullptr};
  int col_every = 0, col_slot = 0, col_count = 0;
  double* hyp = nullptr;
  bool dev_scalars = false;
  double* pin_hyp = nullptr;
  double* gsum_v = nullptr; bool w_part_gsum = false;
  double* gpart_w = nullptr; int ngp_w = 0;
  double* gpart_v = nullptr; int ngp_v = 0;
  bool fuse_gram = true;
  bool curve = false, curve_opt = true;
  std::vector<unsigned char> cv_cij;
  int* cv_cptr = nullptr; int* cv_crow = nullptr; double* cv_cdef = nullptr;
  int* cv_rptr = nullptr; int* cv_rcol = nullptr; double* cv_rdef = nullptr;
  double* eig_cols = nullptr;
  int* cv_dcols = nullptr; int cv_ndef = 0;
  bool w_part_curve = false;
  bool split_accum = false;
  bool w_local_done = false, v_local_done = false;
  int w_local_rpb = 0, w_local_mode = 0, v_local_rpb = 0, v_local_mode = 0;
  hipEvent_t ev_draw = nullptr, ev_join = nullptr;
  ncclComm_t comm = nullptr; int comm_rank = 0, comm_world = 1, gather_rank = 0, gather_world = 1;
  bool comm_rehearse = false;
  hipStream_t comm_stream = nullptr;
  double* comm_scr = nullptr; size_t comm_scr_elems = 0;
  double* comm_words = nullptr;
  btf::PeerMailbox* peer_box = nullptr;
  btf::PeerTable* peer_tab = nullptr;
  unsigned* peer_counters = nullptr;
  std::vector<void*> peer_opened;
  bool peer_on = false;
  unsigned long long peer_epoch = 0;
  long long peer_timeout_ticks = 0;
  bool tau_pending = false; unsigned long long tau_seed = 0; double tau_stability = 1e-6;
  bool fused_sweep = true;
  double* sse_cols = nullptr; bool sse_cols_valid = false;
  double* vs_rec = nullptr; size_t vs_rec_elems = 0;
  bool nu2_drawn_since_v = false;
  bool sc_pending = false; unsigned long long sc_seed = 0; int sc_which = 0; double sc_prior[4] = {0, 0, 0, 0};
  bool lam_pending = false; unsigned long long lam_seed = 0; int lam_exact = 0;
  bool band_in_wsolve = true;
  bool v_wants_band = false, band_img = false; int band_PB = 0;
  bool lam_in_wsolve = true;
  unsigned long long sweep_w = 0, sweep_v = 0;
  int fused_dataflow = 1;
  int fused_step = 1;
  unsigned* fz_words = nullptr; int fz_tiles_w = 0, fz_tiles_v = 0;
  double* fz_pub = nullptr;
  unsigned fz_epoch = 0, fz_gram_total = 0, fz_w_total = 0;
  bool profiling = false;
  std::vector<btf::EvPair> ev_pool;
  size_t ev_used = 0;
  double ms_total[BTF_K_COUNT] = {0};
  int64_t launches[BTF_K_COUNT] = {0};
  std::string err;
  int fail_index = -1;
};

namespace btf {
inline int fail(btf_ctx* c, int code, const std::string& msg) { return report_error(c, code, msg); }

#define HIPCHK(ctx, call)                                                                  \
  do {                                                                                     \
    hipError_t e__ = (call);                                                               \
    if (e__ != hipSuccess)                                                                 \
      return fail(ctx, BTF_EHIP, std::string(#call) + ": " + hipGetErrorString(e__));      \
  } while (0)

template <typename T>
inline int dev_alloc(btf_ctx* c, T** p, size_t n) {
  if (*p) { (void)hipFree(*p); *p = nullptr; }
  if (n == 0) n = 1;
  HIPCHK(c, hipMalloc((void**)p, n * sizeof(T)));
  return BTF_OK;
}

void launch_summary(Scratch& s, const double* W, const double* V, int S, int rows, int MT, int K, int transform, const double* dq,
                    int nq, double* mean, double* quant);
int fold_fail_index();
inline int use_device(int device) {
  const hipError_t e = hipSetDevice(device);
  return e == hipSuccess ? BTF_OK : fail(nullptr, BTF_EHIP, std::string("hipSetDevice: ") + hipGetErrorString(e));
}

struct Prof {
  btf_ctx* c; int kid; EvPair* ev = nullptr;
  Prof(btf_ctx* c_, int kid_) : c(c_), kid(kid_) {
    c->launches[kid]++;
    if (c->profiling && c->ev_used < c->ev_pool.size()) {
      ev = &c->ev_pool[c->ev_used++];
      ev->kid = kid;
    }
  }
  template <typename F, typename... Args>
  void launch(F kernel, dim3 grid, dim3 block, size_t lds, Args... args) {
    launch_on(c->stream, kernel, grid, block, lds, args...);
  }
// ... 57 lines not shown
```

### functionalmf_amd/csrc/btf_fused.h

```cpp
#pragma once
#include "btf_kernels.h"
#include "btf_spectral.h"

namespace btf {

__device__ __forceinline__ bool poll_flag(const unsigned* flag, unsigned epoch) {
  for (unsigned spins = 0; spins < (1u << 22); ++spins) {
    if (__hip_atomic_load((const gu32_t*)flag, __ATOMIC_RELAXED, __HIP_MEMORY_SCOPE_AGENT) == epoch) return true;
    __builtin_amdgcn_s_sleep(8);
  }
  return false;
}

struct HypPub { const double* pub; const unsigned* flag; unsigned epoch; int which; };

struct FuseW {
  WSolveArgs a;
  unsigned* cnt;
  unsigned expected;
  int owners;
  int rows;
  int rw;
  HypPub hp;
  const unsigned* gram_cnt; unsigned gram_expected;
// ... 193 lines not shown
#pragma unroll
  for (int r = 0; r < K; ++r) {
    const bool fresh = live && ok && r < d;
    if (fresh) a.W[(size_t)i * K + r] = y[r];
    wrow[r] = fresh ? y[r] : 0.0;
  }
  if (live && (d < K || !ok)) {
#pragma unroll
    for (int r = 0; r < K; ++r)
      if (!(ok && r < d)) wrow[r] = a.W[(size_t)i * K + r];
  }
  }
  if (!a.gout) return;
  __syncthreads();
  if (solver) {
#pragma unroll
    for (int r = 0; r < K; ++r) stg[r * R + threadIdx.x] = wrow[r];
  }
  __syncthreads();
  {
    typedef double v4f64_w __attribute__((ext_vector_type(4)));
    const int kk = lane >> 4, ii = lane & 15;
    const int nlt = a.nl - r0;
    for (int vbl = wave; vbl < R / RW; vbl += WAVES) {
      if (vbl * RW < nlt) {
        const double* src = stg + (ii < K ? ii : 0) * R + vbl * RW + kk;
        v4f64_w acc = {0.0, 0.0, 0.0, 0.0};
        for (int sidx = 0; sidx < RW / 4; ++sidx) {
          const double x = ii < K ? src[4 * sidx] : 0.0;
          acc = __builtin_amdgcn_mfma_f64_16x16x4f64(x, x, acc, 0, 0, 0);
        }
        const int vb = r0 / RW + vbl;
#pragma unroll
        for (int r = 0; r < 4; ++r) {
          const int row = 4 * r + kk;
          if (row < K && ii <= row) a.gout[(size_t)vb * KK + lidx(row, ii)] = acc[r];
        }
      }
    }
  }
  TAIL_STAMP(stamps, 7);
}

struct FuseV {
  VSpecArgs a;
  unsigned* cnt;
  const double* eig_pub;
  const unsigned* eig_flag; unsigned epoch;
  HypPub hp;
  int band_early;
  int dataflow;
  const unsigned long long* eig_gran;
  const double* pimg;
};
template <> __device__ __forceinline__ unsigned* fuse_tickets<FUSE_V>(const FuseV& fz) { return fz.cnt; }
template <> __device__ __forceinline__ int fuse_chunks<FUSE_V>(const FuseV& fz) { return fz.a.nch; }
template <> __device__ __forceinline__ int fuse_owners<FUSE_V>(const FuseV&) { return 0; }
constexpr int VF_GROUP_WAVES = 4;
constexpr int VF_MAILBOX = 128;
template <> struct FusePre<FUSE_V> { typedef struct VPre type; };
template <> struct FusePre<FUSE_VDF> { typedef struct VPre type; };
static_assert(VF_MAILBOX == VF_MAILBOX_DOUBLES, "mailbox");
#ifndef BTF_VF_BANDPRE
#define BTF_VF_BANDPRE 1
#endif
#if BTF_VF_BANDPRE
struct VPre { double pv[2]; };
#else
struct VPre { int se0, se1; int srow[VS_MAXE]; double scf[VS_MAXE]; double tau[2]; };
#endif
__host__ __device__ inline int vf_band_doubles(int T, int TF, int nD) { return ((nD + 1) & ~1) + 2 * (((T + TF + 2) * (TF + 2) + 1) & ~1); }
__host__ __device__ inline int vf_top_base(int T, int TF, int nD, bool unr3) {
  return vf_red_doubles(unr3) - VF_MAILBOX - (ACC_TILE / T) * vf_band_doubles(T, TF, nD);
}
__host__ __device__ constexpr int vf_cols_per_tile(int T) { return (T == 32 || T == 64 || T == 128) ? ACC_TILE / T : 0; }
__host__ __device__ inline int vf_col_stride(int T, int K, int TF, int nD) { return (vs_layout(T, K, TF, nD, false).total + 1) & ~1; }
__host__ __device__ inline bool vf_fits(int T, int K, int TF, int nD, int waves, bool unr3) {
  const int ng = vf_cols_per_tile(T);
  if (!(ng > 0 && ng * VF_GROUP_WAVES <= waves && nD <= 2 * VF_GROUP_WAVES * WAVE && K + K * K + 8 <= VF_MAILBOX)) return false;
  const int top = vf_top_base(T, TF, nD, unr3);
  return ng * vf_col_stride(T, K, TF, nD) <= top && 16 * 6 * ACC_TILE <= top;
}

#if BTF_VF_BANDPRE
template <int K, int S>
__device__ __forceinline__ bool v_fused_band_preload(const FuseV& fv, int tile, VPre& pre) {
  pre.pv[0] = pre.pv[1] = 0.0;
  const VSpecArgs& a = fv.a;
  if (!a.pband) return false;
  const int T = a.T, NG = ACC_TILE / T;
  const int lane = threadIdx.x & 63;
  const int pw = __builtin_amdgcn_readfirstlane(threadIdx.x >> 6);
  const int cg = pw % NG, wave = pw / NG, tid = wave * WAVE + lane;
  const int j = tile * NG + cg;
  constexpr int NT = VF_GROUP_WAVES * WAVE;
  if (wave < VF_GROUP_WAVES && j < a.ml) {
#pragma unroll
    for (int u = 0; u < 2; ++u)
      if (tid + u * NT < T * (S + 1)) pre.pv[u] = a.pband[(size_t)j * T * (S + 1) + tid + u * NT];
  }
  return true;
}
template <int K, int S>
__device__ __forceinline__ void v_fused_band_store(const FuseV& fv, int tile, double* lds, const VPre& pre, bool unr3) {
  const VSpecArgs& a = fv.a;
  const int T = a.T, NG = ACC_TILE / T;
// ... 447 lines not shown
  DfWork W;
  int o = 0;
  W.mraw = o; o += T * K;
  W.mt = o; o += K * (T + S + 1);
  o = (o + 1) & ~1;
  W.rz = o; o += 2 * T * K;
  W.head = o; o += 2 * K * 4;
  W.gs = o; o += VS_THREADS;
  W.stride = (o + 3) & ~3;
  return W;
}
__host__ __device__ inline bool vf_df_fits(int T, int K, int TF, int nD, int waves, int rg) {
  const int ng = vf_cols_per_tile(T);
  if (!(ng > 0 && ng * VF_GROUP_WAVES <= waves && K <= rg && K + K * K <= 96 && TF == 2)) return false;
  if (waves != 16) return false;
  if (2 * df_layout(T, K, TF + 1).PB > 2 * 8 * WAVE) return false;
  const int nwt = ((waves - ng) / ng) * WAVE;
  if (T * K > nwt || T * K > 768) return false;
  const int room = vf_red_doubles(false) - VF_MAILBOX - ng * df_layout(T, K, TF + 1).size;
  return waves * K * ACC_TILE + ng * df_work(T, K, TF + 1).stride <= room;
}
template <> __device__ __forceinline__ int fuse_chain_waves<FUSE_VDF>(const FuseV& fz) { return ACC_TILE / fz.a.T; }
template <> __device__ __forceinline__ const unsigned* fuse_eig_flag<FUSE_VDF>(const FuseV& fz) { return fz.eig_flag; }
template <> __device__ __forceinline__ const double* fuse_eig_pub<FUSE_VDF>(const FuseV& fz) { return fz.eig_pub; }
template <> __device__ __forceinline__ unsigned fuse_epoch<FUSE_VDF>(const FuseV& fz) { return fz.epoch; }
template <> __device__ __forceinline__ unsigned* fuse_tickets<FUSE_VDF>(const FuseV& fz) { return nullptr; }
template <> __device__ __forceinline__ int fuse_chunks<FUSE_VDF>(const FuseV& fz) { return 1; }
template <> __device__ __forceinline__ int fuse_owners<FUSE_VDF>(const FuseV&) { return 0; }

__device__ __forceinline__ void df_signal(unsigned* c) {
  __builtin_amdgcn_fence(__ATOMIC_RELEASE, "workgroup");
  if ((threadIdx.x & 63) == 0) __hip_atomic_fetch_add(c, 1u, __ATOMIC_RELAXED, __HIP_MEMORY_SCOPE_WORKGROUP);
}
#ifndef BTF_DF_SLEEP
#define BTF_DF_SLEEP 1
#endif
template <int SLEEP = BTF_DF_SLEEP>
__device__ __forceinline__ void df_wait(unsigned* c, unsigned target, unsigned* bad) {
  bool seen = false;
  for (unsigned spins = 0; spins < (1u << 22) / SLEEP; ++spins) {
    if (__hip_atomic_load(c, __ATOMIC_RELAXED, __HIP_MEMORY_SCOPE_WORKGROUP) >= target) { seen = true; break; }
    __builtin_amdgcn_s_sleep(SLEEP);
  }
  if (!seen && (threadIdx.x & 63) == 0) __hip_atomic_store(bad, 1u, __ATOMIC_RELAXED, __HIP_MEMORY_SCOPE_WORKGROUP);
  __builtin_amdgcn_fence(__ATOMIC_ACQUIRE, "workgroup");
}

template <int K, int S>
__device__ __forceinline__ void v_df_begin(const FuseV& fv, int tile, double* lds, VDfPre& pre) {
  unsigned* cw = reinterpret_cast<unsigned*>(lds + vf_red_doubles(false) - VF_MAILBOX + 96);
  if (threadIdx.x < 64) cw[threadIdx.x] = 0u;
  __syncthreads();
  v_df_band_load<K, S>(fv, tile, pre);
}
template <int K, int S>
__device__ __forceinline__ void v_df_band_load(const FuseV& fv, int tile, VDfPre& pre) {
  const VSpecArgs& a = fv.a;
  const int T = a.T, NG = ACC_TILE / T;
  const int lane = threadIdx.x & 63;
  const int pw = __builtin_amdgcn_readfirstlane(threadIdx.x >> 6);
  const int cg = pw - NG, j = tile * NG + cg;
#pragma unroll
  for (int u = 0; u < 8; ++u) pre.pv[u] = make_double2(0.0, 0.0);
  if (pw >= NG && pw < 2 * NG && j < a.ml) {
    const int PB = df_layout(T, K, S).PB;
    const double2* src = reinterpret_cast<const double2*>(fv.pimg + (size_t)j * 2 * PB);
#pragma unroll
    for (int u = 0; u < 8; ++u)
      if (lane + 64 * u < PB) pre.pv[u] = src[lane + 64 * u];
  }
}
template <int K, int S>
__device__ __forceinline__ void v_df_band_store(const FuseV& fv, int tile, double* lds, const VDfPre& pre) {
  const VSpecArgs& a = fv.a;
  const int T = a.T, NG = ACC_TILE / T;
  const int lane = threadIdx.x & 63;
  const int pw = __builtin_amdgcn_readfirstlane(threadIdx.x >> 6);
  const int cg = pw - NG;
  if (!(pw >= NG && pw < 2 * NG && tile * NG + cg < a.ml)) return;
  const DfLayout D = df_layout(T, K, S);
  double2* dst = reinterpret_cast<double2*>(lds + vf_red_doubles(false) - VF_MAILBOX - (size_t)(cg + 1) * D.size + D.P);
#pragma unroll
  for (int u = 0; u < 8; ++u)
    if (lane + 64 * u < D.PB) dst[lane + 64 * u] = pre.pv[u];
  unsigned* cw = reinterpret_cast<unsigned*>(lds + vf_red_doubles(false) - VF_MAILBOX + 96);
  df_signal(cw + DFC_GROUP0 + cg * DFC_PER_GROUP + DFG_BAND);
}

template <int K, int S, int WAVES, int RG, int NVV>
__device__ __forceinline__ void v_fused_df(const FuseV& fv, int tile, double* lds, const double (&acc)[NVV][2], long long* stamps,
                                           const DfEarly& early) {
  static_assert(NVV == K && K <= RG, "one reduction round");
  static_assert(S == 3 && WAVES == 16, "tf_order 2, 16 waves");
  VSpecArgs a = fv.a;
  const int T = a.T, n = T * K, KK = tri(K);
  constexpr int D1 = S + 1, WN = S * (S + 1) + S;
  constexpr int NT = VF_GROUP_WAVES * WAVE;
  const int NG = ACC_TILE / T;
  const int Tp = T + S + 1;
  int nl, nr, ns;
  spectral_split(T, S, nl, nr, ns);
  const int lane = threadIdx.x & 63;
  const int pw = __builtin_amdgcn_readfirstlane(threadIdx.x >> 6);
  const int lgNG = T == 128 ? 0 : (T == 64 ? 1 : 2);
  const int cg = pw & (NG - 1), vw = pw >> lgNG;
  const int j = tile * NG + cg, jg = a.col0 + j;
  const bool live = j < a.ml;
  const int NSW = WAVES;
  const int NWK = (WAVES - NG) >> lgNG;
  const int wk = vw - 1;
  const int first_worker = NG;
  const DfLayout D = df_layout(T, K, S);
  const DfWork Wk = df_work(T, K, S);
  double* mailbox = lds + vf_red_doubles(false) - VF_MAILBOX;
  unsigned* cw = reinterpret_cast<unsigned*>(mailbox + 96);
  unsigned* cgw = cw + DFC_GROUP0 + cg * DFC_PER_GROUP;
  double* top = lds + vf_red_doubles(false) - VF_MAILBOX - (size_t)(cg + 1) * D.size;
  double* P = top + D.P;
  double* Pm = top + D.Pm;
  double* Q = top + D.Q;
  double* win = top + D.win;
  double* flag = top + D.flag;
  double* base = lds + (size_t)NSW * K * ACC_TILE + (size_t)cg * Wk.stride;
  double* mraw = base + Wk.mraw;
  double* mt = base + Wk.mt;
  double* rz = base + Wk.rz;
  double* head = base + Wk.head;
  const double* gsh = mailbox;
  const double* Ush = mailbox + K;
  if (a.hyp && a.hyp_noise) {
    const double nu2 = a.hyp[HYP_NU2];
    a.s = 1.0 / nu2; a.sR = a.s * a.Rrep;
  }

  if (vw == 0) {
#pragma unroll
    for (int v = 0; v < K; ++v)
      *reinterpret_cast<double2*>(&lds[((size_t)pw * K + v) * ACC_TILE + 2 * lane]) = make_double2(acc[v][0], acc[v][1]);
    df_signal(cw + DFC_PART);
    if (!live) return;
    const int nchain = nr > 0 ? 2 * K : K;
    const bool chain = lane < nchain;
    const int side = lane >= K ? 1 : 0;
    const int k = chain ? lane - side * K : 0;
    for (int i0 = 2 * lane; i0 < n; i0 += 2 * WAVE) {
      double z0, z1;
      if (a.z) { const double2 zz = *reinterpret_cast<const double2*>(a.z + (size_t)jg * n + i0); z0 = zz.x; z1 = zz.y; }
      else philox_normal_pair(a.seed, a.stream, ((unsigned long long)jg * n + i0) >> 1, z0, z1);
      rz[(size_t)i0 * 2 + 1] = z0;
      if (i0 + 1 < n) rz[(size_t)(i0 + 1) * 2 + 1] = z1;
    }
    unsigned long long ghi = 0ULL, glo = 0ULL;
    bool okw = false;
    for (unsigned spins = 0; !okw && spins < (1u << 20); ++spins) {
      ghi = __hip_atomic_load(fv.eig_gran + 2 * k, __ATOMIC_RELAXED, __HIP_MEMORY_SCOPE_AGENT);
      glo = __hip_atomic_load(fv.eig_gran + 2 * k + 1, __ATOMIC_RELAXED, __HIP_MEMORY_SCOPE_AGENT);
      okw = __all((unsigned)ghi == fv.epoch && (unsigned)glo == fv.epoch) != 0;
      if (!okw) __builtin_amdgcn_s_sleep(4);
    }
    if (!okw && lane == 0) {
      __hip_atomic_store(cw + DFC_BAD, 1u, __ATOMIC_RELAXED, __HIP_MEMORY_SCOPE_WORKGROUP);
      if (atomicCAS(&a.status[0], 0, 2) == 0) a.status[1] = -1;
    }
    const double g0 = okw ? __longlong_as_double((long long)(((ghi >> 32) << 32) | (glo >> 32))) : 1.0;
    df_wait(cgw + DFG_BAND, 1u, cw + DFC_BAD);
    TAIL_STAMP(stamps, 3);
    const double* Pv = side ? Pm : P;
    double* cq = Q + (size_t)(k * T + (side ? nl : 0)) * 4;
    const int n_elim = side ? nr : nl;
    const int n_common = nr > 0 ? (nl < nr ? nl : nr) : nl;
    double shift = 0.0, eps = a.eps0;
    int tried = 0;
    bool ok;
    double gk;
    while (true) {
      bool good = true;
      gk = fma(g0, a.sR, shift);
      {
        double c[S + 1][S + 1];
#pragma unroll
        for (int b = 0; b < S; ++b) {
          const double2 p0 = *reinterpret_cast<const double2*>(Pv + b * 4), p1 = *reinterpret_cast<const double2*>(Pv + b * 4 + 2);
          c[b][0] = p0.x + gk; c[b][1] = p0.y; c[b][2] = p1.x; c[b][3] = p1.y;
        }
        bool bad = false;
        auto pivot = [&](int i) {
          const double2 p0 = *reinterpret_cast<const double2*>(Pv + (i + S) * 4), p1 = *reinterpret_cast<const double2*>(Pv + (i + S) * 4 + 2);
          c[S][0] = p0.x + gk; c[S][1] = p0.y; c[S][2] = p1.x; c[S][3] = p1.y;
          const double d0 = c[0][0];
          bad |= !(d0 > 0.0);
          const double inv = rcp_cubic(d0);
          double l[S + 1];
#pragma unroll
          for (int d = 1; d <= S; ++d) l[d] = c[0][d] * inv;
#pragma unroll
          for (int b = 1; b <= S; ++b)
#pragma unroll
// ... 265 lines not shown
```

### functionalmf_amd/csrc/btf_kernels.h

```cpp
#pragma once
#include <type_traits>
#include "btf_device.h"
#include "btf_eig.h"
#include "btf_pg_exact.h"

namespace btf {

#ifndef BTF_ACC_WAVES
#define BTF_ACC_WAVES 16
#endif
#ifndef BTF_DF_UNR
#define BTF_DF_UNR 4
#endif
#ifndef BTF_DF_PREFETCH
#define BTF_DF_PREFETCH 1
#endif
#ifndef BTF_DF_SHARE
#define BTF_DF_SHARE 0
#endif
#ifndef BTF_ACC_UNR
#define BTF_ACC_UNR 2
#endif
#ifndef BTF_ACC_PF_WT
#define BTF_ACC_PF_WT 0
// ... 209 lines not shown
#define BTF_ACC_LEAN_EU 0
#endif
__host__ __device__ constexpr int acc_eu_min(int K, int MODE, int FUSE) { return (FUSE == 4 && BTF_ACC_LEAN_EU > 0) ? BTF_ACC_LEAN_EU : ((K >= 10 && MODE == 0 && BTF_ACC_K10_EU > 0) ? BTF_ACC_K10_EU : 1); }
__host__ __device__ constexpr int acc_eu_max(int K, int MODE, int FUSE) { return (FUSE == 4 && BTF_ACC_LEAN_EU > 0) ? BTF_ACC_LEAN_EU : ((K >= 10 && MODE == 0 && BTF_ACC_K10_EU > 0) ? BTF_ACC_K10_EU : 8); }
#if BTF_ACC_K10_EU > 0 || BTF_ACC_LEAN_EU > 0
#define BTF_ACC_EU_ATTR(K, MODE, WAVES, FUSE) __attribute__((amdgpu_waves_per_eu(acc_eu_min(K, MODE, FUSE), acc_eu_max(K, MODE, FUSE))))
#else
#define BTF_ACC_EU_ATTR(K, MODE, WAVES, FUSE)
#endif
#ifndef BTF_ACC_OPL1_MINK
#define BTF_ACC_OPL1_MINK 9
#endif
__host__ __device__ constexpr int acc_opl(int K, int MODE) { return MODE >= 1 && K >= BTF_ACC_OPL1_MINK ? 1 : 2; }
template <int NW> __device__ void sweep_scalar_side(const ScalarSide& sc, double* red);
template <int NW> __device__ void sweep_lam_side(const LamSide& lm, double* red);

enum { FUSE_NONE = 0, FUSE_W = 1, FUSE_V = 2, FUSE_VDF = 3, FUSE_LEAN = 4 };
struct FuseNone {};
struct FuseW;
struct FuseV;
template <int FUSE> struct FuseSel { typedef FuseNone type; };
template <> struct FuseSel<FUSE_W> { typedef FuseW type; };
template <> struct FuseSel<FUSE_V> { typedef FuseV type; };
template <> struct FuseSel<FUSE_VDF> { typedef FuseV type; };
template <> struct FuseSel<FUSE_LEAN> { typedef FuseNone type; };
template <int K, int WAVES> __device__ __forceinline__ void w_fused_owner(const FuseW& fw, int tile, double* lds, long long* stamps);
template <int FUSE> __device__ __forceinline__ int fuse_owners(const typename FuseSel<FUSE>::type& fz);
struct VPre;
template <int K, int S, int WAVES, int NSUM>
__device__ __forceinline__ void v_fused_tail(const FuseV& fv, int tile, double* lds, const double (&sums)[NSUM], int nv_round, int tv, int tc, long long* stamps,
                                             const VPre& pre, const double* mailbox, bool band_early, bool unr3);
template <int K, int S> __device__ __forceinline__ void v_fused_prefetch(const FuseV& fv, int tile, double* mailbox, VPre& pre, bool band_early);
template <int K, int S, class PRE> __device__ __forceinline__ void v_fused_prefetch_loads(const FuseV& fv, int tile, PRE& pre, bool band_early);
constexpr int VF_PRE = 4;
template <int K, int S> __device__ __forceinline__ bool v_fused_band_early(const FuseV& fv, int tile, double* lds, bool unr3);
#ifndef BTF_VF_BANDPRE
#define BTF_VF_BANDPRE 1
#endif
#if BTF_VF_BANDPRE
template <int K, int S> __device__ __forceinline__ bool v_fused_band_preload(const FuseV& fv, int tile, VPre& pre);
template <int K, int S> __device__ __forceinline__ void v_fused_band_store(const FuseV& fv, int tile, double* lds, const VPre& pre, bool unr3);
#endif
template <int FUSE> struct FusePre { struct type {}; };
constexpr int VF_MAILBOX_DOUBLES = 128;
struct VDfPre { double2 pv[8]; };
template <int FUSE> __device__ __forceinline__ int fuse_chain_waves(const typename FuseSel<FUSE>::type& fz) { return 0; }
struct DfEarly { double epub; bool have; };
template <int FUSE> __device__ __forceinline__ const unsigned* fuse_eig_flag(const typename FuseSel<FUSE>::type& fz) { return nullptr; }
template <int FUSE> __device__ __forceinline__ const double* fuse_eig_pub(const typename FuseSel<FUSE>::type& fz) { return nullptr; }
template <int FUSE> __device__ __forceinline__ unsigned fuse_epoch(const typename FuseSel<FUSE>::type& fz) { return 0u; }
template <int K, int S> __device__ __forceinline__ void v_df_begin(const FuseV& fv, int tile, double* lds, VDfPre& pre);
template <int K, int S> __device__ __forceinline__ void v_df_band_load(const FuseV& fv, int tile, VDfPre& pre);
template <int K, int S> __device__ __forceinline__ void v_df_band_store(const FuseV& fv, int tile, double* lds, const VDfPre& pre);
template <int K, int S, int WAVES, int RG, int NVV>
__device__ __forceinline__ void v_fused_df(const FuseV& fv, int tile, double* lds, const double (&acc)[NVV][2], long long* stamps, const DfEarly& early);
template <int FUSE> __device__ __forceinline__ unsigned* fuse_tickets(const typename FuseSel<FUSE>::type& fz);
template <int FUSE> __device__ __forceinline__ int fuse_chunks(const typename FuseSel<FUSE>::type& fz);
__device__ __forceinline__ bool last_arriver_of(unsigned* cnt, unsigned expected, unsigned* word) {
  if (threadIdx.x == 0) {
    const unsigned t = __hip_atomic_fetch_add((gu32_t*)cnt, 1u, __ATOMIC_RELAXED, __HIP_MEMORY_SCOPE_AGENT);
    const bool last = t + 1u == expected;
    if (last) __hip_atomic_store((gu32_t*)cnt, 0u, __ATOMIC_RELAXED, __HIP_MEMORY_SCOPE_AGENT);
    *word = last ? 1u : 0u;
  }
  __syncthreads();
  const bool last = *word != 0u;
  __syncthreads();
  return last;
}
__host__ __device__ constexpr int vf_red_doubles(bool unr3) { return unr3 ? 15360 : 18432; }
__host__ __device__ constexpr int w_tail_lds_doubles(int K);
__host__ __device__ constexpr int w_owner_lds_budget(int K);

#ifdef BTF_ACC_STAMPS
#define ACC_STAMP(i) do { if (threadIdx.x == 0 && b < 4096 && cm.stamps) cm.stamps[b * 8 + (i)] = wall_clock64(); } while (0)
#define ACC_SIDE_STAMP(i) do { if (threadIdx.x == 0 && cm.stamps) cm.stamps[(4096 + blockIdx.x) * 8 + (i)] = wall_clock64(); } while (0)
#define ACC_TAIL_STAMPS (cm.stamps && b < 4096 ? cm.stamps + b * 8 : nullptr)
#define ACC_OWNER_STAMPS (cm.stamps ? cm.stamps + (size_t)(4096 + blockIdx.x) * 8 : nullptr)
#else
#define ACC_STAMP(i) do { } while (0)
#define ACC_SIDE_STAMP(i) do { } while (0)
#define ACC_TAIL_STAMPS nullptr
#define ACC_OWNER_STAMPS nullptr
#endif
#define TAIL_STAMP(st, i) do { if ((st) && threadIdx.x == 0) (st)[i] = wall_clock64(); } while (0)
template <int K, int MODE, int WAVES = acc_waves(K, MODE), typename CT = double, typename XT = double, int UNRV = 0,
          int OPL = acc_opl(K, MODE), int FUSE = FUSE_NONE>
__global__ __launch_bounds__(WAVES * WAVE) BTF_ACC_EU_ATTR(K, MODE, WAVES, FUSE) void accum_kernel(
    const XT* __restrict__ X, const CT* __restrict__ Cx, const double* __restrict__ U,
    const int* __restrict__ srcmap, double* __restrict__ part, int Rdim, int ld,
    int rows_per_block, EigSide side, EigSideCols sidec, TauSide tau, GramSide gram, ChunkMap cm, SweepSide sw,
    typename FuseSel<FUSE>::type fz) {
  static_assert(FUSE == FUSE_NONE || (MODE == 0 && OPL == 2 && WAVES == 16), "the fused tails follow the complete-data stream");
  constexpr bool PLAIN = FUSE == FUSE_NONE || FUSE == FUSE_LEAN;
  constexpr int KK = tri(K);
  constexpr int NV = MODE == 0 ? K : K + KK;
  constexpr int ACC_WAVES = WAVES;
  constexpr int ACC_UNR = FUSE == FUSE_VDF ? BTF_DF_UNR : (UNRV > 0 ? UNRV : (MODE >= 1 ? BTF_ACC_UNR_WT : (K >= 9 ? BTF_ACC_UNR_K9 : BTF_ACC_UNR)));
  constexpr int ACC_RGT = WAVES * WAVE / ACC_TILE, ACC_RGL = (96 * 1024) / (WAVES * ACC_TILE * 8);
  constexpr int ACC_RG0 = ACC_RGT < 4 ? ACC_RGT : 4;
  constexpr int ACC_RGW = ACC_RGT < ACC_RGL ? (ACC_RGT < NV ? ACC_RGT : NV) : (ACC_RGL < NV ? ACC_RGL : NV);
  constexpr int ACC_RG = ACC_RGW > ACC_RG0 ? ACC_RGW : ACC_RG0;
  constexpr int RED_SLOT = ACC_RG * ACC_TILE;
  constexpr int RED_SLOTS = (FUSE == FUSE_V || FUSE == FUSE_VDF) ? (vf_red_doubles(UNRV == 3) + RED_SLOT - 1) / RED_SLOT : ACC_WAVES;
  static_assert(RED_SLOTS >= ACC_WAVES, "reduction scratch");
  __shared__ double red[RED_SLOTS][ACC_RG][ACC_TILE];
// ... 94 lines not shown
        drain_stores();
        __syncthreads();
        if (threadIdx.x == 0) __hip_atomic_fetch_add((gu32_t*)gram.cnt, 1u, __ATOMIC_RELAXED, __HIP_MEMORY_SCOPE_AGENT);
      }
      ACC_SIDE_STAMP(3);
      return;
    }
    b -= gram.nblocks;
  }
  if (gram.sum_src) {
    if (b == 0) {
      double* scratch = &red[0][0][0];
      const int lanes = gram.sum_threads / KK > 32 ? 32 : (gram.sum_threads / KK < 1 ? 1 : gram.sum_threads / KK);
      const int l = threadIdx.x / KK, q = threadIdx.x - l * KK;
      if ((int)threadIdx.x < gram.sum_threads && l < lanes) {
        double sg = 0.0;
        for (int b0 = l; b0 < gram.sum_n; b0 += 8 * lanes) {
          double x[8];
#pragma unroll
          for (int u = 0; u < 8; ++u) x[u] = b0 + u * lanes < gram.sum_n ? gram.sum_src[(size_t)(b0 + u * lanes) * KK + q] : 0.0;
#pragma unroll
          for (int u = 0; u < 8; ++u) sg += x[u];
        }
        scratch[l * KK + q] = sg;
      }
      __syncthreads();
      if ((int)threadIdx.x < KK) {
        double t = 0.0;
        for (int bb = 0; bb < lanes; ++bb) t += scratch[bb * KK + threadIdx.x];
        gram.sum_out[threadIdx.x] = t;
      }
      return;
    }
    b -= 1;
  }
  return;
  }
  b -= cm.nside;
  ACC_STAMP(0);
  const int ntiles = ld / ACC_TILE;
  const int lchunk = b / ntiles, tile = b - lchunk * ntiles;
  const int chunk = cm.slot_base + lchunk;
  static_assert(OPL == 2 || (OPL == 1 && WAVES % 2 == 0), "outputs per lane");
  constexpr int NWR = OPL == 2 ? WAVES : WAVES / 2;
  const int half = OPL == 2 ? 0 : (wave & 1);
  const int wv = OPL == 2 ? wave : (wave >> 1);
  const size_t col = (size_t)tile * ACC_TILE + (OPL == 2 ? 2 * lane : 64 * half + lane);
  int r0 = cm.row_base + lchunk * rows_per_block;
  if (r0 >= cm.skip_at) r0 += cm.skip_rows;
  const int r1 = min(r0 + rows_per_block, cm.row_end);

  constexpr bool dataflow = FUSE == FUSE_VDF;
  static_assert(!dataflow || (UNRV != 3 && NV <= ACC_RG && OPL == 2), "the dataflow tail: one reduction round, two rows in flight");
  bool df_band_done = false;
  DfEarly df_early{0.0, false};
  VDfPre dfpre;
  if constexpr (dataflow) v_df_begin<K, 3>(fz, tile, &red[0][0][0], dfpre);
  int df_ncw = 0;
  if constexpr (dataflow) df_ncw = fuse_chain_waves<FUSE>(fz);
  int nwr_rt = NWR;
  bool band_early = false;
  if constexpr (FUSE == FUSE_V) band_early = v_fused_band_early<K, 3>(fz, tile, &red[0][0][0], UNRV == 3);
  typename FusePre<FUSE>::type vpre;
#if BTF_VF_BANDPRE
  if constexpr (FUSE == FUSE_V) band_early = v_fused_band_preload<K, 3>(fz, tile, vpre);
#endif
  double acc[NV][OPL];
#pragma unroll
  for (int v = 0; v < NV; ++v)
#pragma unroll
    for (int o = 0; o < OPL; ++o) acc[v][o] = 0.0;
#ifdef BTF_NO_NT
  constexpr bool nt = false;
#else
  const bool nt = __builtin_amdgcn_readfirstlane(cm.nt) != 0;
#endif
  int s0 = 0, s1 = 0;
  bool gram_on = true, gram_any = true;
  if constexpr (MODE == 2) {
    s0 = srcmap[col];
    if constexpr (OPL == 2) s1 = srcmap[col + 1];
    const bool own = s0 == (int)col || (OPL == 2 && s1 == (int)col + 1);
    gram_on = __builtin_amdgcn_readfirstlane(__any(own) ? 1 : 0) != 0;
    if constexpr (OPL == 1) gram_any = __syncthreads_or(own ? 1 : 0) != 0;
    else gram_any = gram_on;
  }
  int cs_form = 0, cs_src = 0;
  if constexpr (MODE == 2 && OPL == 2) {
    cs_src = __builtin_amdgcn_readfirstlane(s0);
    if (__all(s0 == cs_src && s1 == cs_src)) cs_form = 1;
    else if (__all(s1 == s0 + 1 && (s0 & 1) == 0)) cs_form = 2;
    cs_form = __builtin_amdgcn_readfirstlane(cs_form);
  }

  int ublk0 = r0;
  struct Rows { double2 x[ACC_UNR]; double2 c[MODE >= 1 ? ACC_UNR : 1]; double2 cs[MODE == 2 ? ACC_UNR : 1]; double uk[ACC_UNR][K]; };
  auto load_rows = [&](int rb, Rows& R, auto full, auto ntc) {
    constexpr bool FULL = decltype(full)::value;
    constexpr bool NT = decltype(ntc)::value;
#pragma unroll
    for (int u = 0; u < ACC_UNR; ++u) {
      const int r = rb + u * (dataflow ? nwr_rt : NWR);
      if constexpr (ULDS) {
        const double* up = ush + (size_t)((FULL ? r : min(r, r1 - 1)) - ublk0) * K;
#pragma unroll
        for (int k = 0; k < K; ++k) R.uk[u][k] = up[k];
      } else {
// ... 83 lines not shown
        double2* dst = reinterpret_cast<double2*>(ush);
        const int n2 = (bend - ublk0) * K / 2;
        for (int i = threadIdx.x; i < n2; i += WAVES * WAVE) dst[i] = src[i];
        if (((bend - ublk0) * K & 1) && threadIdx.x == 0) ush[(bend - ublk0) * K - 1] = U[(size_t)bend * K - 1];
      }
      __syncthreads();
      if (ublk0 == r0) ACC_STAMP(1);
      const int bfull = min(full_end, bend - (ACC_UNR - 1) * NWR);
      for (; rb < bfull; rb += STEP) {
        Rows A;
        load_rows(rb, A, std::true_type{}, ntc);
        compute(rb, A);
      }
      if (rb < bend) {
        Rows A;
        load_rows(rb, A, std::false_type{}, ntc);
        compute(rb, A);
        rb += STEP;
      }
    }
  } else if constexpr (PIPELINED) {
    Rows A, B;
    bool more = rb < full_end;
    if (more) load_rows(rb, A, std::true_type{}, ntc);
    while (more) {
      const bool nextB = rb + STEP < full_end;
      if (nextB) load_rows(rb + STEP, B, std::true_type{}, ntc);
      compute(rb, A);
      rb += STEP;
      if (!nextB) break;
      more = rb + STEP < full_end;
      if (more) load_rows(rb + STEP, A, std::true_type{}, ntc);
      compute(rb, B);
      rb += STEP;
    }
  } else {
    if constexpr (FUSE == FUSE_V) {
      const int pre_end = full_end - VF_PRE * STEP;
      for (; rb < pre_end; rb += STEP) {
        Rows A;
        load_rows(rb, A, std::true_type{}, ntc);
        compute(rb, A);
      }
      v_fused_prefetch_loads<K, 3>(fz, tile, vpre, band_early);
    }
    if constexpr (dataflow) {
      const int g1 = NWR * ACC_UNR;
      const int rsplit = r0 + ((r1 - r0) * BTF_DF_SHARE / 100) / g1 * g1;
      nwr_rt = NWR;
      for (rb = r0 + wv; rb < rsplit; rb += g1) {
        Rows A;
        load_rows(rb, A, std::true_type{}, ntc);
        compute(rb, A);
        if (!df_band_done) { v_df_band_store<K, 3>(fz, tile, &red[0][0][0], dfpre); df_band_done = true; }
      }
      if (wave >= df_ncw) {
        nwr_rt = NWR - df_ncw;
        const int step = nwr_rt * ACC_UNR, fend = r1 - (ACC_UNR - 1) * nwr_rt;
        const bool eigw = BTF_DF_PREFETCH && wave == df_ncw;
        const int rprobe = r0 + (r1 - r0) * 5 / 8;
        unsigned eflag = 0u;
        int estate = 0;
        for (rb = rsplit + wv - df_ncw; rb < fend; rb += step) {
          Rows A;
          load_rows(rb, A, std::true_type{}, ntc);
          if (eigw && estate < 2 && rb >= rprobe) {
            if (estate == 1 && eflag == fuse_epoch<FUSE>(fz)) {
              if (lane < K + K * K) df_early.epub = load_sc1(fuse_eig_pub<FUSE>(fz) + lane);
              df_early.have = true;
              estate = 2;
            } else {
              eflag = __hip_atomic_load(fuse_eig_flag<FUSE>(fz), __ATOMIC_RELAXED, __HIP_MEMORY_SCOPE_AGENT);
              estate = 1;
            }
          }
          compute(rb, A);
          if (!df_band_done) { v_df_band_store<K, 3>(fz, tile, &red[0][0][0], dfpre); df_band_done = true; }
        }
        if (rb < r1) {
          Rows A;
          load_rows(rb, A, std::false_type{}, ntc);
          compute(rb, A);
        }
      }
      rb = r1;
    }
    for (; rb < full_end; rb += STEP) {
      Rows A;
      load_rows(rb, A, std::true_type{}, ntc);
      compute(rb, A);
    }
  }
  if constexpr (!ULDS) {
    if (rb < r1) {
      Rows A;
      load_rows(rb, A, std::false_type{}, ntc);
      compute(rb, A);
    }
  }

  };
  if (nt) run_stream(std::true_type{}); else run_stream(std::false_type{});
  ACC_STAMP(2);
  if constexpr (dataflow) {
    if (!df_band_done) {
      v_df_band_load<K, 3>(fz, tile, dfpre);
      v_df_band_store<K, 3>(fz, tile, &red[0][0][0], dfpre);
    }
    v_fused_df<K, 3, WAVES, ACC_RG, NV>(fz, tile, &red[0][0][0], acc, ACC_TAIL_STAMPS, df_early);
    return;
  }
  if constexpr (FUSE == FUSE_V) {
    if constexpr (ULDS) v_fused_prefetch_loads<K, 3>(fz, tile, vpre, band_early);
#if BTF_VF_BANDPRE
    if (band_early) v_fused_band_store<K, 3>(fz, tile, &red[0][0][0], vpre, UNRV == 3);
#endif
    v_fused_prefetch<K, 3>(fz, tile, &red[0][0][0] + RED_SLOTS * RED_SLOT - VF_MAILBOX_DOUBLES, vpre, band_early);
  }
  const int tv = threadIdx.x >> 7;
  const int tc = threadIdx.x & 127;
  constexpr int NFS = PLAIN ? 1 : (NV + ACC_RG - 1) / ACC_RG;
  double fsum[NFS];
#pragma unroll
  for (int r = 0; r < NFS; ++r) fsum[r] = 0.0;
#pragma unroll
  for (int g = 0; g < NV; g += ACC_RG) {
    if (MODE == 2 && !gram_any && g >= K) break;
#pragma unroll
    for (int v = 0; v < ACC_RG; ++v) {
      if (g + v < NV) {
        if constexpr (OPL == 2) *reinterpret_cast<double2*>(&red[wave][v][2 * lane]) = make_double2(acc[g + v][0], acc[g + v][1]);
        else red[wv][v][64 * half + lane] = acc[g + v][0];
      }
    }
    __syncthreads();
    if constexpr (!ULDS) { if (g == 0) ACC_STAMP(1); }
    if (tv < ACC_RG && g + tv < NV && !(MODE == 2 && !gram_on && g + tv >= K)) {
      double s = 0.0;
#pragma unroll
      for (int w = 0; w < NWR; ++w) s += red[w][tv][tc];
      if constexpr (PLAIN) {
#ifdef BTF_PART_SC1
        store_sc1(&part[((size_t)chunk * NV + (g + tv)) * ld + (size_t)tile * ACC_TILE + tc], s);
#else
        part[((size_t)chunk * NV + (g + tv)) * ld + (size_t)tile * ACC_TILE + tc] = s;
#endif
      } else {
        if (FUSE == FUSE_W || fuse_tickets<FUSE>(fz)) store_sc1(&part[((size_t)chunk * NV + (g + tv)) * ld + (size_t)tile * ACC_TILE + tc], s);
        if constexpr (FUSE == FUSE_V) fsum[g / ACC_RG] = s;
      }
    }
    __syncthreads();
  }
  ACC_STAMP(3);
  if constexpr (FUSE == FUSE_W) {
    drain_stores();
    __syncthreads();
// ... 65 lines not shown
__device__ inline void reduce_gram(const double* __restrict__ gpart, int ngp, int KK, double scale,
                                   double* scratch, double* G) {
  const int lanes = gram_lanes(KK);
  const int l = threadIdx.x / KK, q = threadIdx.x - l * KK;
  double s = 0.0;
  if (l < lanes) {
    for (int b0 = l; b0 < ngp; b0 += 8 * lanes) {
      double x[8];
#pragma unroll
      for (int u = 0; u < 8; ++u) x[u] = b0 + u * lanes < ngp ? gpart[(size_t)(b0 + u * lanes) * KK + q] : 0.0;
#pragma unroll
      for (int u = 0; u < 8; ++u) s += x[u];
    }
  }
  reduce_gram_tail(s, KK, scale, scratch, G);
}

__device__ __forceinline__ bool gram_early_ok(int ngp, int KK) { return ngp <= 8 * gram_lanes(KK); }
__device__ __forceinline__ void reduce_gram_fetch(const double* __restrict__ gpart, int ngp, int KK, double (&x)[8]) {
  const int lanes = gram_lanes(KK);
  const int l = threadIdx.x / KK, q = threadIdx.x - l * KK;
#pragma unroll
  for (int u = 0; u < 8; ++u) x[u] = (l < lanes && l + u * lanes < ngp) ? gpart[(size_t)(l + u * lanes) * KK + q] : 0.0;
}
__device__ inline void reduce_gram_finish(const double (&x)[8], int ngp, int KK, double scale, double* scratch, double* G) {
  double s = 0.0;
#pragma unroll
  for (int u = 0; u < 8; ++u) s += x[u];
  reduce_gram_tail(s, KK, scale, scratch, G);
}

template <int K>
__global__ __launch_bounds__(WAVE) void colgram_kernel(const double* __restrict__ V, int T, int ncols, double* __restrict__ out) {
  constexpr int KK = tri(K);
  const int j = blockIdx.x, lane = threadIdx.x;
  if (j >= ncols) return;
  double acc[KK];
#pragma unroll
  for (int q = 0; q < KK; ++q) acc[q] = 0.0;
  for (int t = lane; t < T; t += WAVE) {
    double v[K];
#pragma unroll
    for (int k = 0; k < K; ++k) v[k] = V[((size_t)j * T + t) * K + k];
#pragma unroll
    for (int a = 0; a < K; ++a)
#pragma unroll
      for (int b = 0; b <= a; ++b) acc[lidx(a, b)] = fma(v[a], v[b], acc[lidx(a, b)]);
  }
#pragma unroll
  for (int q = 0; q < KK; ++q) {
    const double t = wave_sum(acc[q]);
    if (lane == 0) out[(size_t)j * KK + q] = t;
  }
}

struct WSolveArgs {
  const double* part; int nch; int ld;
  const int* gsrc;
  const double* gpart; int ngp;
  int weighted;
  double s;
  double sR;
  double inv_sigma2;
  double* W; int row0; int nl;
  const double* z; unsigned long long seed; unsigned long long stream;
  int* status;
  double* gout;
  const double* hyp;
  double Rrep;
  int hyp_noise;
  CurveLists cv;
  const double* cv_blocks;
  int nside;
  LamSide lam;
  BandSide band;
#ifdef BTF_WS_STAMPS
  long long* dbg;
#endif
};
#ifdef BTF_WS_STAMPS
#define WS_STAMP(n) do { if (threadIdx.x == 0 && a.dbg) a.dbg[(size_t)blockIdx.x * 6 + (n)] = (long long)__builtin_amdgcn_s_memtime(); } while (0)
#else
#define WS_STAMP(n) do {} while (0)
#endif

__device__ inline void band_side(const BandSide& bs, int j, double* itau, int nthreads) {
  const double* tau = bs.Tau2 + (size_t)(bs.col0 + j) * bs.nD;
  double tv[2] = {1.0, 1.0};
  int p0[2] = {0, 0}, p1[2] = {0, 0};
#pragma unroll
  for (int u = 0; u < 2; ++u) {
    const int r = threadIdx.x + u * nthreads, e0 = threadIdx.x + u * nthreads;
    if (r < bs.nD) tv[u] = tau[r];
    if (e0 < bs.TD1) { p0[u] = bs.st_ptr[e0]; p1[u] = bs.st_ptr[e0 + 1]; }
  }
  double lam2 = bs.hyp ? bs.hyp[HYP_LAM2] : bs.lam2;
  if (bs.lam_flag) {
    __shared__ int okf;
    if (threadIdx.x == 0) {
      bool seen = false;
      for (unsigned spins = 0; spins < (1u << 22); ++spins) {
        if (__hip_atomic_load((const gu32_t*)bs.lam_flag, __ATOMIC_RELAXED, __HIP_MEMORY_SCOPE_AGENT) == bs.epoch) { seen = true; break; }
        __builtin_amdgcn_s_sleep(8);
      }
      okf = seen ? 1 : 0;
      if (!seen && atomicCAS(&bs.status[0], 0, 2) == 0) bs.status[1] = -2;
    }
    __syncthreads();
    if (!okf) return;
    lam2 = load_sc1(bs.lam_pub + HYP_LAM2);
  }
#pragma unroll
  for (int u = 0; u < 2; ++u) {
    const int r = threadIdx.x + u * nthreads;
    if (r < bs.nD) itau[r] = 1.0 / __dmul_rn(lam2, tv[u]);
  }
  __syncthreads();
#pragma unroll
  for (int u = 0; u < 2; ++u) {
    const int e0 = threadIdx.x + u * nthreads;
    if (e0 < bs.TD1) {
      double s = 0.0;
      for (int e = p0[u]; e < p1[u]; ++e) s = fma(bs.st_coef[e], itau[bs.st_row[e]], s);
      bs.pband[(size_t)j * bs.TD1 + e0] = s;
      if (bs.pimg) {
        const int t = e0 / bs.img_D1, d = e0 - t * bs.img_D1;
        double* im = bs.pimg + (size_t)j * 2 * bs.img_PB;
        im[e0] = s;
// ... 10 lines not shown
#define BTF_WS_SPLIT_U 4
#endif
__host__ __device__ constexpr int ws_split_of(int K, bool weighted) { return weighted ? ws_split(K) : (K <= 6 ? BTF_WS_SPLIT_U : ws_split(K)); }
__host__ __device__ constexpr size_t ws_gram_stage(int K, bool weighted) {
  return (size_t)ws_split_of(K, weighted) * (K + tri(K)) * WS_ROWS;
}

__host__ __device__ constexpr int ws_rows_for(int nl) { return nl > 2048 ? 64 : (nl > 1024 ? 32 : (nl > 512 ? 16 : 8)); }

constexpr int WS_CHB = 32;
template <bool SC1 = false>
__device__ __forceinline__ double chunk_sum_seq(const double* __restrict__ p, size_t cst, int nch) {
  double s = 0.0;
  int c = 0;
  for (; c + WS_CHB <= nch; c += WS_CHB) {
    double x[WS_CHB];
#pragma unroll
    for (int u = 0; u < WS_CHB; ++u) x[u] = SC1 ? load_sc1(p + (size_t)(c + u) * cst) : p[(size_t)(c + u) * cst];
#pragma unroll
    for (int u = 0; u < WS_CHB; ++u) s += x[u];
  }
  if (c < nch) {
    double x[WS_CHB];
#pragma unroll
    for (int u = 0; u < WS_CHB; ++u) x[u] = c + u < nch ? (SC1 ? load_sc1(p + (size_t)(c + u) * cst) : p[(size_t)(c + u) * cst]) : 0.0;
#pragma unroll
    for (int u = 0; u < WS_CHB; ++u) if (c + u < nch) s += x[u];
  }
  return s;
}

template <int K, bool WEIGHTED, int RW = WS_ROWS>
__global__ __launch_bounds__(WS_ROWS * ws_split_of(K, WEIGHTED)) void w_solve_kernel(WSolveArgs a) {
  constexpr int KK = tri(K);
  constexpr int SUB = WS_ROWS / RW;
  constexpr int WS_SPLIT = ws_split_of(K, WEIGHTED);
  constexpr int NVMAX = WEIGHTED ? K + KK : K;
  constexpr int NV = NVMAX;
  WS_STAMP(0);
  constexpr int UNR = WEIGHTED ? (K + KK > 24 ? 1 : 2) : 4;
  __shared__ double G[KK];
  __shared__ double red[WS_SPLIT][K + KK][WS_ROWS];
  __shared__ double zsh[K][WS_ROWS];
  __shared__ double cvq[WEIGHTED ? 1 : RW][WEIGHTED ? 1 : KK];
  const int lane = threadIdx.x & 63, grp = threadIdx.x >> 6;
  if (a.nside) {
    const int nsolve = (int)gridDim.x - a.nside;
    if ((int)blockIdx.x >= nsolve) {
      int b = (int)blockIdx.x - nsolve;
      if (a.lam.hyp) {
        if (b == 0) { sweep_lam_side<WS_ROWS * WS_SPLIT / WAVE>(a.lam, &red[0][0][0]); return; }
        --b;
      }
      if (a.band.pband && b < a.band.ml) band_side(a.band, b, &red[0][0][0], WS_ROWS * WS_SPLIT);
      return;
    }
  }
  if constexpr (!WEIGHTED) {
    if (a.cv.ptr) {
      constexpr int NT = WS_ROWS * WS_SPLIT, G = NT / KK, CAP = (WS_SPLIT * (K + KK) * WS_ROWS) / KK;
      const int i0 = a.row0 + blockIdx.x * RW, i1 = min(i0 + RW, a.row0 + a.nl);
      const int e0 = a.cv.ptr[i0], e1 = a.cv.ptr[i1];
      double* stage = &red[0][0][0];
      const int g = threadIdx.x / KK, q = threadIdx.x - g * KK;
      if (g < G)
        for (int r = g; r < RW; r += G) cvq[r][q] = 0.0;
      for (int eb = e0; eb < e1; eb += CAP) {
        const int ee = min(eb + CAP, e1);
        if (g < G) {
          for (int e = eb + g; e < ee; e += G)
            stage[(size_t)(e - eb) * KK + q] = a.cv.def[e] * a.cv_blocks[(size_t)a.cv.idx[e] * KK + q];
        }
        __syncthreads();
        if (g < G) {
          for (int r = g; r < RW && i0 + r < i1; r += G) {
            double acc = cvq[r][q];
            for (int e = max(a.cv.ptr[i0 + r], eb); e < min(a.cv.ptr[i0 + r + 1], ee); ++e) acc += stage[(size_t)(e - eb) * KK + q];
            cvq[r][q] = acc;
          }
        }
        __syncthreads();
      }
    }
  }
  if (a.hyp) {
    if (a.hyp_noise) { a.s = 1.0 / a.hyp[HYP_NU2]; a.sR = a.s * a.Rrep; }
    a.inv_sigma2 = 1.0 / a.hyp[HYP_SIGMA2];
  }
  double gx[8];
  bool g_early = false;
  if constexpr (!WEIGHTED) {
    g_early = gram_early_ok(a.ngp, KK);
    if (g_early) reduce_gram_fetch(a.gpart, a.ngp, KK, gx);
    else reduce_gram(a.gpart, a.ngp, KK, a.sR, &red[0][0][0], G);
  }
  const int rr = lane % RW, sub = lane / RW;
  const int il = blockIdx.x * RW + rr;
  constexpr int CS = WS_SPLIT * SUB;
  if constexpr (!WEIGHTED) {
    constexpr int NT = WS_ROWS * WS_SPLIT;
    const size_t cst = (size_t)NV * a.ld;
    for (int t = threadIdx.x; t < RW * K; t += NT) {
      const int v = t / RW, r = t - v * RW;
      const int ilr = blockIdx.x * RW + r;
      red[0][v][r] = ilr < a.nl ? chunk_sum_seq(a.part + (size_t)v * a.ld + ilr, cst, a.nch) : 0.0;
    }
    for (int t = NT - 1 - (int)threadIdx.x; t < RW * K; t += NT) {
// ... 2004 lines not shown
```

### include/btf.h

```cpp
#ifndef BTF_H_
#define BTF_H_

#include <stdint.h>

#ifdef __cplusplus
extern "C" {
#endif

typedef struct btf_ctx btf_ctx;

enum {
  BTF_OK = 0,
  BTF_EINVAL = 1,
  BTF_EHIP = 2,
  BTF_ENOTPD = 3,
  BTF_ESTATE = 4
};

enum { BTF_COMPAT_REFERENCE = 0, BTF_COMPAT_EXACT = 1 };

enum {
  BTF_K_STATS = 0,
  BTF_K_W_ACCUM = 1,
  BTF_K_W_SOLVE = 2,
// ... 39 lines not shown

int btf_set_shard(btf_ctx* ctx, int row0, int nrows_local, int col0, int ncols_local);
int btf_set_shard_halo(btf_ctx* ctx, int halo_row, int halo_col);
void* btf_stream(btf_ctx* ctx);
int btf_comm_fork(btf_ctx* ctx, void* comm_stream);
int btf_comm_join(btf_ctx* ctx, void* comm_stream);
#define BTF_COMM_ID_BYTES 128
#define BTF_PEER_DESC_BYTES 256
int btf_peer_export(btf_ctx* ctx, unsigned char* desc, int nbytes);
int btf_peer_init(btf_ctx* ctx, int rank, int world, const unsigned char* descs, int nbytes);
int btf_comm_unique_id(unsigned char* id, int nbytes);
int btf_comm_block(int n, int rank, int world, int32_t* lo, int32_t* len);
int btf_comm_init(btf_ctx* ctx, int rank, int world, const unsigned char* id, int nbytes);
int btf_comm_rehearse(btf_ctx* ctx, int rank, int world);
int btf_comm_destroy(btf_ctx* ctx);
int btf_comm_info(btf_ctx* ctx, int32_t* out);
int btf_allgather_W(btf_ctx* ctx);
int btf_allgather_V(btf_ctx* ctx);
int btf_allreduce_sse(btf_ctx* ctx);
int btf_allreduce_sum(btf_ctx* ctx, double* vals, int n);
int btf_set_gathered_W(btf_ctx* ctx, const double* W);
int btf_set_gathered_V(btf_ctx* ctx, const double* V);
void* btf_dev_W(btf_ctx* ctx);
void* btf_dev_V(btf_ctx* ctx);

int btf_set_data_gaussian(btf_ctx* ctx, const double* y_rows, const double* y_cols, int nreps);
int btf_set_data_binomial(btf_ctx* ctx, const double* succ_rows, const double* trials_rows,
                          const double* succ_cols, const double* trials_cols);
int btf_set_stale_sources(btf_ctx* ctx, const int32_t* src_row, const int32_t* src_col);

int btf_set_data_counts(btf_ctx* ctx, const double* counts, int nreps);
int btf_nb_loglik(btf_ctx* ctx, const double* R, const double* cand, const int32_t* shared3, double* ll);
int btf_nb_set_rate(btf_ctx* ctx, const double* R, const int32_t* shared3);
int btf_nb_mh(btf_ctx* ctx, uint64_t seed, int nsteps, double rpropstdev, double rstdev, const int32_t* shared3,
              const double* R_in);
int btf_nb_get_rate(btf_ctx* ctx, double* R, const int32_t* shared3);

int btf_set_W(btf_ctx* ctx, const double* W);
int btf_get_W(btf_ctx* ctx, double* W);
int btf_set_V(btf_ctx* ctx, const double* V);
int btf_get_V(btf_ctx* ctx, double* V);
int btf_set_hyper(btf_ctx* ctx, const double* Tau2 , double lam2, double sigma2);
int btf_set_tau_chain(btf_ctx* ctx, const double* Tau2_a, const double* Tau2_b, const double* Tau2_c);
int btf_get_tau(btf_ctx* ctx, double* Tau2, double* Tau2_a, double* Tau2_b, double* Tau2_c);
int btf_resample_Tau2(btf_ctx* ctx, uint64_t seed, double lam2, double stability, double* lsum_out );
int btf_queue_Tau2(btf_ctx* ctx, uint64_t seed, double stability);
int btf_queue_lam2(btf_ctx* ctx, uint64_t seed, int compat);
int btf_queue_scalars(btf_ctx* ctx, uint64_t seed, int which, double nu2_a, double nu2_b, double sigma2_a, double sigma2_b,
                      int32_t* queued);

int btf_gibbs_sweeps(btf_ctx* ctx, int nsweeps, uint64_t seed_base, uint64_t draws0, int compat, double nu2_a, double nu2_b,
                     double sigma2_a, double sigma2_b, double stability, double eps0, int attempts);
int btf_wv_steps(btf_ctx* ctx, int n, uint64_t seed_base, uint64_t draws0, int compat, double eps0, int attempts);
int btf_set_nu2(btf_ctx* ctx, double nu2);
void* btf_dev_hyp(btf_ctx* ctx);
int btf_set_global_nobs(btf_ctx* ctx, double nobs);
int btf_set_scalar_slot(btf_ctx* ctx, int slot, double value);
int btf_device_scalars(btf_ctx* ctx, int enable);
int btf_set_scalars(btf_ctx* ctx, double nu2, double sigma2, double lam2, double lam2_a);
int btf_get_scalars(btf_ctx* ctx, double* out6);
int btf_draw_scalars(btf_ctx* ctx, uint64_t seed, int which, double nu2_a, double nu2_b, double sigma2_a, double sigma2_b);
int btf_draw_lam2(btf_ctx* ctx, uint64_t seed, int compat);
int btf_set_omega(btf_ctx* ctx, const double* omega_rows, const double* omega_cols);
int btf_get_omega(btf_ctx* ctx, double* omega_rows);

int btf_w_accum(btf_ctx* ctx, int compat);
int btf_resample_W(btf_ctx* ctx, const double* z, uint64_t seed, int compat);
int btf_resample_V(btf_ctx* ctx, const double* z, uint64_t seed, int compat,
                   double eps0, int attempts);
int btf_get_V_attempts(btf_ctx* ctx, int32_t* tries );
int btf_get_V_order(btf_ctx* ctx, int32_t* order );
int btf_sym_eig(int device, int nembeds, int nparts, const double* parts, double* out, const double* warm_from);

int btf_read_probe(int device, size_t bytes, int reps, double* gb_per_s);
enum { BTF_LIK_COMPLETE = 0, BTF_LIK_WEIGHTED = 1, BTF_LIK_CURVE_COUNTS = 2 };
int btf_get_likelihood_form(btf_ctx* ctx, int32_t* form);
int btf_get_draw_counters(btf_ctx* ctx, uint64_t* w_half_sweeps, uint64_t* v_half_sweeps);
int btf_set_draw_counters(btf_ctx* ctx, uint64_t w_half_sweeps, uint64_t v_half_sweeps);
int btf_get_accum_bytes_per_cell(btf_ctx* ctx, double* bytes);

int btf_set_option(btf_ctx* ctx, int option, int value);
int btf_get_V_sampler(btf_ctx* ctx, int32_t* which);

int btf_sse(btf_ctx* ctx, double* sse, double* nobs);
int btf_sse_begin(btf_ctx* ctx);
int btf_sse_end(btf_ctx* ctx, double* sse, double* nobs, double* W_out);
int btf_pg_draw(btf_ctx* ctx, uint64_t seed);

int btf_pg_batch(int device, int64_t n, const double* b, const double* psi, uint64_t seed, double* out);
int btf_pg_batch_mode(int device, int64_t n, const double* b, const double* psi, uint64_t seed, int mode, double* out);

int btf_sync(btf_ctx* ctx);
int btf_host_selftest(void);

int btf_mvn_banded(int device, int batch, int n, int bw, const double* band,
                   const double* mu_part, const double* z, uint64_t seed,
                   double eps0, int attempts, double* x_out, int32_t* tries_out);

enum { BTF_MVN_PRECISION = 1, BTF_MVN_FACTOR = 2 };
int btf_mvn_dense(int device, int batch, int n, const double* A, int form, const double* mu, const double* mu_part,
                  const double* z, uint64_t seed, double eps0, int attempts, double* x_out, int32_t* tries_out);

#define BTF_ESS_HOST_LIKELIHOOD (-1)
int btf_set_likelihood_param(btf_ctx* ctx, int link, double parameter);
int btf_set_likelihood_table(btf_ctx* ctx, int link, const double* shape, const double* scale, const double* prob, int G);
int btf_set_data_logsum(btf_ctx* ctx, const double* y_rows, const double* y_cols, int nreps);
// ... 128 lines not shown
```

Before: 27020 sweeps/s.

## Predraw V-step Gaussian noise in W-solve side blocks for dataflow V kernel

During the W solve, extra side blocks generate the Philox normal draws that the following V update will need, writing them to a device buffer keyed by seed, sweep and shape. The fused dataflow V kernel then loads these predrawn values into LDS instead of generating the normals inline on its critical path. This moves RNG work into idle capacity of the W-solve launch, at the cost of an extra global buffer write and read plus bookkeeping to invalidate stale draws.

```diff
diff --git a/functionalmf_amd/_native.py b/functionalmf_amd/_native.py
--- a/functionalmf_amd/_native.py
+++ b/functionalmf_amd/_native.py
@@ -148,6 +148,8 @@
     "btf_gibbs_sweeps": (C.c_int, [_ctx, C.c_int, C.c_uint64, C.c_uint64, C.c_int, C.c_double, C.c_double, C.c_double,
                                    C.c_double, C.c_double, C.c_double, C.c_int]),
     "btf_wv_steps": (C.c_int, [_ctx, C.c_int, C.c_uint64, C.c_uint64, C.c_int, C.c_double, C.c_int]),
+    "btf_announce_V_seed": (C.c_int, [_ctx, C.c_uint64]),
+    "btf_get_predrawn_info": (C.c_int, [_ctx, C.POINTER(C.c_int64)]),
     "btf_gass_set_constraints": (C.c_int, [_ctx, _c_dp, C.c_int, _c_dp, C.c_int]),
     "btf_gass_begin": (C.c_int, [_ctx, C.c_int, C.c_int, _c_dp, _c_dp, C.c_uint64, C.c_double, C.c_int, C.c_int]),
     "btf_gass_grid": (C.c_int, [_ctx, C.c_int, _c_ip, C.POINTER(C.c_uint8), _c_dp, _c_dp]),
diff --git a/functionalmf_amd/csrc/btf_abi.hip b/functionalmf_amd/csrc/btf_abi.hip
--- a/functionalmf_amd/csrc/btf_abi.hip
+++ b/functionalmf_amd/csrc/btf_abi.hip
@@ -210,6 +210,8 @@
         constexpr int RG = K < 4 ? 4 : (K > 6 ? 6 : K);
         f2.dataflow = (df_on && f2.a.pband && f2.pimg && !f2.cnt && !f2.hp.flag && K <= 6 &&
                        vf_df_fits(f2.a.T, K, f2.a.TF, f2.a.nD, 16, RG)) ? 1 : 0;
+        if (!f2.dataflow || f2.a.z) f2.zpre = nullptr;
+        if (f2.zpre) ++c->zpre_used;
 
         if constexpr (K <= 6) {
           if (f2.dataflow) { p.launch(accum_kernel<K, 0, 16, double, double, 0, 2, FUSE_VDF>, grid, dim3(16 * WAVE), 0, X, Cx, U, srcmap, c->part, Rdim, ld, rpb, side, sidec, tau, gram, cm, sw, f2); return; }
@@ -286,7 +288,8 @@
   Prof p(c, BTF_K_W_SOLVE);
   WSolveArgs a = a0;
   const int rw = ws_rows_for(a.nl);
-  a.nside = (a.lam.hyp ? 1 : 0) + (a.band.pband ? a.band.ml : 0);
+  const int nth = WS_ROWS * ws_split_of(K, a.weighted != 0);
+  a.nside = (a.lam.hyp ? 1 : 0) + (a.band.pband ? a.band.ml : 0) + (a.zs.out ? (a.zs.npairs + nth - 1) / nth : 0);
   const dim3 grid((a.nl + rw - 1) / rw + a.nside);
 #define WS_LAUNCH(WT, RWV) p.launch(w_solve_kernel<K, WT, RWV>, grid, dim3(WS_ROWS * ws_split_of(K, WT)), 0, a)
 #define WS_PICK(WT) do { if (rw == 8) WS_LAUNCH(WT, 8); else if (rw == 16) WS_LAUNCH(WT, 16); else if (rw == 32) WS_LAUNCH(WT, 32); else WS_LAUNCH(WT, 64); } while (0)
@@ -713,6 +716,7 @@
   { const char* e = std::getenv("BTF_LAM_IN_WSOLVE"); if (e) c->lam_in_wsolve = std::atoi(e) != 0; }
   { const char* e = std::getenv("BTF_BAND_IN_WSOLVE"); if (e) c->band_in_wsolve = std::atoi(e) != 0; }
   { const char* e = std::getenv("BTF_VF_DATAFLOW"); if (e) c->fused_dataflow = std::atoi(e) != 0 ? 1 : 0; }
+  { const char* e = std::getenv("BTF_PREDRAW"); if (e) c->predraw = std::atoi(e) != 0; }
   if (stream) { c->stream = (hipStream_t)stream; }
   else {
     const hipError_t e = hipStreamCreateWithFlags(&c->stream, hipStreamNonBlocking);
@@ -743,7 +747,7 @@
   if (c->stream) (void)hipStreamSynchronize(c->stream);
   void* ptrs[] = {c->A_wT, c->C_wT, c->A_v, c->C_v, c->B_wT, c->B_v, c->W, c->V, c->Tau2, c->part,
                   c->gpart, c->zbuf, c->bsum, c->gband, c->status, c->tries, c->st_ptr, c->st_row, c->st_coef,
-                  c->srcmap_w, c->srcmap_v, c->pband, c->pimg, c->dbg, c->gpart_w, c->gpart_v, c->gsum_v, c->eig, c->cv_cptr, c->cv_crow, c->cv_cdef, c->cv_rptr, c->cv_rcol, c->cv_rdef, c->eig_cols, c->cv_dcols, c->A8_wT, c->A8_v, c->gs_cons, c->gs_cc, c->gs_rc, c->gs_av, c->gs_mask, c->gs_info, c->gs_thetas, c->gs_ntheta, c->gs_ll, c->gs_llp, c->gs_hh, c->gs_cur, c->gs_nacc, c->gs_u, c->st_drow, c->st_dcoef, c->essX0, c->essNu, c->ess_st, c->ess_theta, c->ess_done, c->ess_part, c->Ta, c->Tb, c->Tc, c->lsum, c->dr_ptr, c->dr_col, c->dr_val, c->sse_cols, c->vs_rec, c->vc_scratch, c->gs_cptr, c->gs_cidx, c->gs_cval,
+                  c->srcmap_w, c->srcmap_v, c->pband, c->pimg, c->dbg, c->gpart_w, c->gpart_v, c->gsum_v, c->eig, c->cv_cptr, c->cv_crow, c->cv_cdef, c->cv_rptr, c->cv_rcol, c->cv_rdef, c->eig_cols, c->cv_dcols, c->A8_wT, c->A8_v, c->gs_cons, c->gs_cc, c->gs_rc, c->gs_av, c->gs_mask, c->gs_info, c->gs_thetas, c->gs_ntheta, c->gs_ll, c->gs_llp, c->gs_hh, c->gs_cur, c->gs_nacc, c->gs_u, c->st_drow, c->st_dcoef, c->essX0, c->essNu, c->ess_st, c->ess_theta, c->ess_done, c->ess_part, c->Ta, c->Tb, c->Tc, c->lsum, c->dr_ptr, c->dr_col, c->dr_val, c->sse_cols, c->vs_rec, c->vc_scratch, c->zpre, c->gs_cptr, c->gs_cidx, c->gs_cval,
                   c->ep_rows, c->ep_cols, c->ep_crow, c->ep_ccol, c->ep_mu, c->ep_corr, c->ep_pband, c->ep_envg, c->ep_f, c->ep_off,
                   c->gg_tab, c->gg_Lw, c->gg_Lv,
                   c->ft_rows, c->ft_cols, c->ft_U, c->ft_side, c->ft_X0, c->ft_Nu, c->ft_z, c->ft_mask, c->ft_info, c->ft_thetas,
@@ -783,6 +787,7 @@
   if (c->pband) { (void)hipFree(c->pband); c->pband = nullptr; c->pband_version = 0; }
   if (c->pimg) { (void)hipFree(c->pimg); c->pimg = nullptr; c->pimg_version = 0; }
   c->v_wants_band = false;
+  c->zpre_rec.drop(); c->v_seed_announced = false;
   c->nb_bwt_written = false;
   return BTF_OK;
 }
@@ -1040,6 +1045,7 @@
   c->ngp_v = 0;
   c->w_local_done = false;
   c->sse_cols_valid = false;
+  c->zpre_rec.drop(); c->v_seed_announced = false;
   return BTF_OK;
 }
 int btf_set_gathered_V(btf_ctx* c, const double* V) {
@@ -1366,6 +1372,9 @@
   const int want_mode = !wt ? 0 : (compat == BTF_COMPAT_REFERENCE && c->stale_w && c->srcmap_w ? 2 : 1);
   int rc;
   c->v_local_done = false;
+  const bool v_announced = c->v_seed_announced;
+  c->v_seed_announced = false;
+  c->zpre_rec.drop();
   const double* dz = nullptr;
   if (z) {
     const size_t nz = (size_t)w_z_offset(c->N, K);
@@ -1419,6 +1428,14 @@
         c->pband_version = c->prior_version;
         c->pimg_version = c->band_img ? c->prior_version : 0;
       }
+    }
+    if (v_announced && c->predraw && whole && !wt && !cv && c->have_hyper && c->fused_step >= 1 && c->fused_dataflow && c->TF == 2 && K <= 6 &&
+        banded_choice(c) == 3 && vf_df_fits(c->T, K, c->TF, c->nD, 16, K < 4 ? 4 : K)) {
+      const size_t nz = (size_t)c->ml * c->T * K;
+      if (nz > c->zpre_elems) { if ((rc = dev_alloc(c, &c->zpre, nz))) return rc; c->zpre_elems = nz; }
+      a.zs = ZSide{c->zpre, c->v_seed_next, 2 * c->sweep_v + 0x10001ULL, ((unsigned long long)c->col0 * c->T * K) >> 1, (int)(nz / 2)};
+      c->zpre_rec.set(c->v_seed_next, c->sweep_v, c->col0, c->ml, c->T, K);
+      ++c->zpre_drawn;
     }
     K_SWITCH(K, launch_wsolve<KT>(c, a));
     c->ngp_w = a.gout ? wblocks : 0;
@@ -1589,6 +1606,8 @@
   c->sse_cols_valid = false;
   struct ResetFlag { bool& f; ~ResetFlag() { f = false; } } reset_nu2_flag{c->nu2_drawn_since_v};
   const int K = c->K, KK = c->KK, T = c->T, n = T * K;
+  const bool z_ahead = !z && c->zpre && c->zpre_rec.matches(seed, c->sweep_v, c->col0, c->ml, T, K);
+  c->zpre_rec.drop();
   const bool wt = lik_weighted(c), cv = c->weighted && !wt;
   const int mode = !wt ? 0 : (compat == BTF_COMPAT_REFERENCE && c->stale_v && c->srcmap_v ? 2 : 1);
   c->v_part_mode = mode;
@@ -1725,6 +1744,7 @@
         side.pub = c->fz_pub + FZ_PUB_EIG; side.flag = c->fz_words + FZ_EIG; side.epoch = c->fz_epoch;
         side.gran = reinterpret_cast<unsigned long long*>(c->fz_pub + FZ_PUB_GRAN);
         fv.eig_gran = side.gran;
+        if (z_ahead) fv.zpre = c->zpre;
         if (sw.lam.hyp) {
           sw.lam.pub = c->fz_pub + FZ_PUB_HYP; sw.lam.flag = c->fz_words + FZ_LAM; sw.lam.epoch = c->fz_epoch;
           fv.hp = HypPub{c->fz_pub + FZ_PUB_HYP, c->fz_words + FZ_LAM, c->fz_epoch, 4};
@@ -2542,6 +2562,7 @@
     if ((rc = btf_queue_scalars(c, d + 3, 3, nu2_a, nu2_b, sigma2_a, sigma2_b, &queued))) return rc;
     if ((rc = btf_w_accum(c, compat))) return rc;
     if (!queued) { if ((rc = btf_draw_scalars(c, d + 3, 7, nu2_a, nu2_b, sigma2_a, sigma2_b))) return rc; }
+    c->v_seed_announced = true; c->v_seed_next = d + 5;
     if ((rc = btf_resample_W(c, nullptr, d + 4, compat))) return rc;
     if ((rc = btf_resample_V(c, nullptr, d + 5, compat, eps0, attempts))) return rc;
     if (c->col_every > 0 && --c->col_count == 0) {
@@ -2560,9 +2581,22 @@
   int rc;
   for (int s = 0; s < n; ++s) {
     const uint64_t d = seed_base + draws0 + 2ULL * (uint64_t)s;
+    c->v_seed_announced = true; c->v_seed_next = d + 2;
     if ((rc = btf_resample_W(c, nullptr, d + 1, compat))) return rc;
     if ((rc = btf_resample_V(c, nullptr, d + 2, compat, eps0, attempts))) return rc;
   }
+  return BTF_OK;
+}
+
+int btf_announce_V_seed(btf_ctx* c, uint64_t seed) {
+  if (!c) return BTF_EINVAL;
+  c->v_seed_announced = true; c->v_seed_next = seed;
+  return BTF_OK;
+}
+
+int btf_get_predrawn_info(btf_ctx* c, int64_t* out) {
+  if (!c || !out) return BTF_EINVAL;
+  out[0] = c->zpre_rec.valid ? 1 : 0; out[1] = c->zpre_drawn; out[2] = c->zpre_used;
   return BTF_OK;
 }
 
@@ -3516,6 +3550,7 @@
 
 int btf_set_option(btf_ctx* c, int option, int value) {
   if (!c) return BTF_EINVAL;
+  c->zpre_rec.drop(); c->v_seed_announced = false;
   switch (option) {
     case BTF_OPT_SAMPLER:
       if (value < BTF_SAMPLER_BANDED || value > BTF_SAMPLER_BANDED_NOPANEL) return fail(c, BTF_EINVAL, "unknown sampler");
@@ -3574,6 +3609,7 @@
 int btf_set_draw_counters(btf_ctx* c, uint64_t w, uint64_t v) {
   if (!c) return BTF_EINVAL;
   c->sweep_w = w; c->sweep_v = v;
+  c->zpre_rec.drop(); c->v_seed_announced = false;
   c->sse_cols_valid = false;
   HIPCHK(c, hipSetDevice(c->dev));
   const size_t rec = (size_t)c->K + (size_t)c->K * c->K + 8;
@@ -4003,6 +4039,19 @@
   ST_CHECK(pg_class_of(33.0, PG_MODE_DEFAULT) == PG_CLASS_SERIES && pg_class_of(33.0, PG_MODE_EXACT_ALL) == PG_CLASS_FLAT);
   ST_CHECK(pg_class_of(2.5, PG_MODE_EXACT_ALL) == PG_CLASS_FRAC && pg_class_of(2.0, PG_MODE_SERIES_ALL) == PG_CLASS_SERIES);
   ST_CHECK(pg_class_of(200.0, PG_MODE_EXACT_ALL) == PG_CLASS_NORMAL);
+  {
+    ZPreRecord r;
+    ST_CHECK(!r.matches(0, 0, 0, 0, 0, 0));
+    r.set(7, 3, 0, 256, 64, 5);
+    ST_CHECK(r.matches(7, 3, 0, 256, 64, 5));
+    ST_CHECK(!r.matches(8, 3, 0, 256, 64, 5) && !r.matches(7, 4, 0, 256, 64, 5) && !r.matches(7, 3, 1, 256, 64, 5));
+    ST_CHECK(!r.matches(7, 3, 0, 255, 64, 5) && !r.matches(7, 3, 0, 256, 32, 5) && !r.matches(7, 3, 0, 256, 64, 6));
+    r.drop();
+    ST_CHECK(!r.matches(7, 3, 0, 256, 64, 5));
+    for (int T : {32, 64, 128})
+      for (int K = 1; K <= 6; ++K)
+        if (vf_df_fits(T, K, 2, T - 3, 16, K < 4 ? 4 : K)) ST_CHECK((T * K) % 2 == 0 && T * K / 2 <= 8 * WAVE);
+  }
 #undef ST_CHECK
   return 0;
 }
diff --git a/functionalmf_amd/csrc/btf_ctx.h b/functionalmf_amd/csrc/btf_ctx.h
--- a/functionalmf_amd/csrc/btf_ctx.h
+++ b/functionalmf_amd/csrc/btf_ctx.h
@@ -15,6 +15,18 @@
 struct PeerMailbox; struct PeerTable;
 constexpr int MAX_K = 10;
 struct EvPair { hipEvent_t a, b; int kid; };
+struct ZPreRecord {
+  bool valid = false;
+  unsigned long long seed = 0, sweep_v = 0;
+  int col0 = 0, ml = 0, T = 0, K = 0;
+  void set(unsigned long long seed_, unsigned long long sweep_v_, int col0_, int ml_, int T_, int K_) {
+    valid = true; seed = seed_; sweep_v = sweep_v_; col0 = col0_; ml = ml_; T = T_; K = K_;
+  }
+  void drop() { valid = false; }
+  bool matches(unsigned long long seed_, unsigned long long sweep_v_, int col0_, int ml_, int T_, int K_) const {
+    return valid && seed == seed_ && sweep_v == sweep_v_ && col0 == col0_ && ml == ml_ && T == T_ && K == K_;
+  }
+};
 }
 
 struct btf_ctx {
@@ -150,6 +162,11 @@
   bool v_wants_band = false, band_img = false; int band_PB = 0;
   bool lam_in_wsolve = true;
   unsigned long long sweep_w = 0, sweep_v = 0;
+  bool v_seed_announced = false; unsigned long long v_seed_next = 0;
+  bool predraw = true;
+  double* zpre = nullptr; size_t zpre_elems = 0;
+  btf::ZPreRecord zpre_rec;
+  long long zpre_drawn = 0, zpre_used = 0;
   int fused_dataflow = 1;
   int fused_step = 1;
   unsigned* fz_words = nullptr; int fz_tiles_w = 0, fz_tiles_v = 0;
diff --git a/functionalmf_amd/csrc/btf_fused.h b/functionalmf_amd/csrc/btf_fused.h
--- a/functionalmf_amd/csrc/btf_fused.h
+++ b/functionalmf_amd/csrc/btf_fused.h
@@ -269,6 +269,7 @@
   int dataflow;
   const unsigned long long* eig_gran;
   const double* pimg;
+  const double* zpre;
 };
 template <> __device__ __forceinline__ unsigned* fuse_tickets<FUSE_V>(const FuseV& fz) { return fz.cnt; }
 template <> __device__ __forceinline__ int fuse_chunks<FUSE_V>(const FuseV& fz) { return fz.a.nch; }
@@ -822,6 +823,34 @@
   if (threadIdx.x < 64) cw[threadIdx.x] = 0u;
   __syncthreads();
   v_df_band_load<K, S>(fv, tile, pre);
+  if (fv.zpre) {
+    const VSpecArgs& a = fv.a;
+    const int NG = ACC_TILE / a.T, n2 = a.T * K / 2;
+    const int lane = threadIdx.x & 63;
+    const int pw = __builtin_amdgcn_readfirstlane(threadIdx.x >> 6);
+    const int j = tile * NG + pw;
+    if (pw < NG && j < a.ml) {
+      const double2* src = reinterpret_cast<const double2*>(fv.zpre + (size_t)j * 2 * n2);
+#pragma unroll
+      for (int u = 0; u < 8; ++u)
+        if (lane + 64 * u < n2) pre.pv[u] = src[lane + 64 * u];
+    }
+  }
+}
+template <int K, int S>
+__device__ __forceinline__ void v_df_z_store(const FuseV& fv, int tile, double* lds, const VDfPre& pre) {
+  if (!fv.zpre) return;
+  const VSpecArgs& a = fv.a;
+  const int T = a.T, NG = ACC_TILE / T, n2 = T * K / 2;
+  const int lane = threadIdx.x & 63;
+  const int pw = __builtin_amdgcn_readfirstlane(threadIdx.x >> 6);
+  if (!(pw < NG && tile * NG + pw < a.ml)) return;
+  double* rz = lds + (size_t)16 * K * ACC_TILE + (size_t)pw * df_work(T, K, S).stride + df_work(T, K, S).rz;
+#pragma unroll
+  for (int u = 0; u < 8; ++u) {
+    const int q = lane + 64 * u;
+    if (q < n2) { rz[(size_t)q * 4 + 1] = pre.pv[u].x; rz[(size_t)q * 4 + 3] = pre.pv[u].y; }
+  }
 }
 template <int K, int S>
 __device__ __forceinline__ void v_df_band_load(const FuseV& fv, int tile, VDfPre& pre) {
@@ -913,6 +942,7 @@
     const bool chain = lane < nchain;
     const int side = lane >= K ? 1 : 0;
     const int k = chain ? lane - side * K : 0;
+    if (!fv.zpre)
     for (int i0 = 2 * lane; i0 < n; i0 += 2 * WAVE) {
       double z0, z1;
       if (a.z) { const double2 zz = *reinterpret_cast<const double2*>(a.z + (size_t)jg * n + i0); z0 = zz.x; z1 = zz.y; }
diff --git a/functionalmf_amd/csrc/btf_kernels.h b/functionalmf_amd/csrc/btf_kernels.h
--- a/functionalmf_amd/csrc/btf_kernels.h
+++ b/functionalmf_amd/csrc/btf_kernels.h
@@ -285,6 +285,7 @@
 template <int K, int S> __device__ __forceinline__ void v_df_begin(const FuseV& fv, int tile, double* lds, VDfPre& pre);
 template <int K, int S> __device__ __forceinline__ void v_df_band_load(const FuseV& fv, int tile, VDfPre& pre);
 template <int K, int S> __device__ __forceinline__ void v_df_band_store(const FuseV& fv, int tile, double* lds, const VDfPre& pre);
+template <int K, int S> __device__ __forceinline__ void v_df_z_store(const FuseV& fv, int tile, double* lds, const VDfPre& pre);
 template <int K, int S, int WAVES, int RG, int NVV>
 __device__ __forceinline__ void v_fused_df(const FuseV& fv, int tile, double* lds, const double (&acc)[NVV][2], long long* stamps, const DfEarly& early);
 template <int FUSE> __device__ __forceinline__ unsigned* fuse_tickets(const typename FuseSel<FUSE>::type& fz);
@@ -485,7 +486,7 @@
 
   constexpr bool dataflow = FUSE == FUSE_VDF;
   static_assert(!dataflow || (UNRV != 3 && NV <= ACC_RG && OPL == 2), "the dataflow tail: one reduction round, two rows in flight");
-  bool df_band_done = false;
+  bool df_band_done = false, df_z_done = false;
   DfEarly df_early{0.0, false};
   VDfPre dfpre;
   if constexpr (dataflow) v_df_begin<K, 3>(fz, tile, &red[0][0][0], dfpre);
@@ -675,7 +676,11 @@
         Rows A;
         load_rows(rb, A, std::true_type{}, ntc);
         compute(rb, A);
-        if (!df_band_done) { v_df_band_store<K, 3>(fz, tile, &red[0][0][0], dfpre); df_band_done = true; }
+        if (!df_band_done) {
+          v_df_band_store<K, 3>(fz, tile, &red[0][0][0], dfpre);
+          v_df_z_store<K, 3>(fz, tile, &red[0][0][0], dfpre);
+          df_band_done = df_z_done = true;
+        }
       }
       if (wave >= df_ncw) {
         nwr_rt = NWR - df_ncw;
@@ -726,6 +731,7 @@
   if (nt) run_stream(std::true_type{}); else run_stream(std::false_type{});
   ACC_STAMP(2);
   if constexpr (dataflow) {
+    if (!df_z_done) v_df_z_store<K, 3>(fz, tile, &red[0][0][0], dfpre);
     if (!df_band_done) {
       v_df_band_load<K, 3>(fz, tile, dfpre);
       v_df_band_store<K, 3>(fz, tile, &red[0][0][0], dfpre);
@@ -897,6 +903,15 @@
     const double t = wave_sum(acc[q]);
     if (lane == 0) out[(size_t)j * KK + q] = t;
   }
+}
+
+struct ZSide { double* out; unsigned long long seed, stream, pair0; int npairs; };
+__device__ __forceinline__ void z_side(const ZSide& zs, int b, int nthreads) {
+  const int p = b * nthreads + (int)threadIdx.x;
+  if (p >= zs.npairs) return;
+  double z0, z1;
+  philox_normal_pair(zs.seed, zs.stream, zs.pair0 + (unsigned long long)p, z0, z1);
+  reinterpret_cast<double2*>(zs.out)[p] = make_double2(z0, z1);
 }
 
 struct WSolveArgs {
@@ -919,6 +934,7 @@
   int nside;
   LamSide lam;
   BandSide band;
+  ZSide zs;
 #ifdef BTF_WS_STAMPS
   long long* dbg;
 #endif
@@ -1035,7 +1051,11 @@
         if (b == 0) { sweep_lam_side<WS_ROWS * WS_SPLIT / WAVE>(a.lam, &red[0][0][0]); return; }
         --b;
       }
-      if (a.band.pband && b < a.band.ml) band_side(a.band, b, &red[0][0][0], WS_ROWS * WS_SPLIT);
+      if (a.band.pband) {
+        if (b < a.band.ml) { band_side(a.band, b, &red[0][0][0], WS_ROWS * WS_SPLIT); return; }
+        b -= a.band.ml;
+      }
+      if (a.zs.out) z_side(a.zs, b, WS_ROWS * WS_SPLIT);
       return;
     }
   }
diff --git a/include/btf.h b/include/btf.h
--- a/include/btf.h
+++ b/include/btf.h
@@ -115,6 +115,8 @@
 int btf_gibbs_sweeps(btf_ctx* ctx, int nsweeps, uint64_t seed_base, uint64_t draws0, int compat, double nu2_a, double nu2_b,
                      double sigma2_a, double sigma2_b, double stability, double eps0, int attempts);
 int btf_wv_steps(btf_ctx* ctx, int n, uint64_t seed_base, uint64_t draws0, int compat, double eps0, int attempts);
+int btf_announce_V_seed(btf_ctx* ctx, uint64_t seed);
+int btf_get_predrawn_info(btf_ctx* ctx, int64_t* out);
 int btf_set_nu2(btf_ctx* ctx, double nu2);
 void* btf_dev_hyp(btf_ctx* ctx);
 int btf_set_global_nobs(btf_ctx* ctx, double nobs);
```

Measured after the change: 26690 sweeps/s. 0.988x the previous value.
